# BaZzz01010101/ReflaxMan

Measured on AMD Instinct MI355X. Metric: Mrays/sec at 3840×2160 depth-8; max per-channel |Δ| vs CPU reference, higher is better.
Workload: dtype f32; 1 GPU; C3 synth16: 16 spheres + 4 textured triangles + sun, 3840x2160, depth 8, 1 spp; scene=synth16, width=3840, height=2160, depth=8, spp=1, parallelism=single-gpu

## Files before the change

include/rfx.h:

```cpp
#ifndef RFX_H
#define RFX_H
#include <stddef.h>
#include <stdint.h>

#ifdef __cplusplus
extern "C" {
#endif

#define RFX_ABI_VERSION 5

typedef enum {
  RFX_OK = 0,
  RFX_ERR_ARG = -1,
  RFX_ERR_HIP = -2,
  RFX_ERR_STATE = -3,
  RFX_ERR_IO = -4,
  RFX_ERR_RNG = -5,
  RFX_ERR_NODEV = -6
} rfx_status;

enum { RFX_METAL = 0, RFX_DIELECTRIC = 1 };

typedef struct rfx_scene rfx_scene;
typedef struct rfx_renderer rfx_renderer;

int rfx_abi_version(void);
const char *rfx_last_error(void);
enum { RFX_BUILD_PRIM_LARGE = 1, RFX_BUILD_PRIM_SSAA = 2, RFX_BUILD_PRIM_LANES = 4, RFX_BUILD_ONE_LIGHT = 8 };
int rfx_build_options(void);

rfx_scene *rfx_scene_create(float diff_r, float diff_g, float diff_b, float diff_power);
void rfx_scene_destroy(rfx_scene *scene);
int rfx_scene_add_sphere(rfx_scene *scene, const float center[3], float radius, int material_type,
                         const float rgb[3], float reflectivity, float transparency);
int rfx_scene_add_triangle(rfx_scene *scene, const float v1[3], const float v2[3], const float v3[3],
                           int material_type, const float rgb[3], float reflectivity, float transparency);
int rfx_scene_add_mesh(rfx_scene *scene, const float *vertices, uint32_t n_vertices, const uint32_t *indices,
                       uint32_t n_triangles, int material_type, const float rgb[3], float reflectivity,
                       float transparency);
int rfx_scene_add_plane(rfx_scene *scene, const float pos[3], const float norm[3], int material_type,
                        const float rgb[3], float reflectivity, float transparency);
int rfx_scene_plane_count(const rfx_scene *scene);
int rfx_triangle_set_texture(rfx_scene *scene, int object_index, int texture_index, const float uv[6]);
int rfx_scene_add_light(rfx_scene *scene, const float origin[3], float radius, const float rgb[3], float power);
int rfx_scene_add_texture_argb(rfx_scene *scene, uint32_t width, uint32_t height, const uint32_t *argb);
int rfx_scene_add_texture_file(rfx_scene *scene, const char *path, int *loaded);
int rfx_scene_set_skybox_file(rfx_scene *scene, const char *path);
int rfx_scene_set_skybox_argb(rfx_scene *scene, uint32_t width, uint32_t height, const uint32_t *argb);
int rfx_scene_counts(const rfx_scene *scene, int *spheres, int *triangles, int *lights, int *textures);
int rfx_scene_tri_bvh_dump(const rfx_scene *scene, int32_t counts[5], float *boxes, int32_t *children,
                           int32_t *leaf_ids, int32_t *residual);
int rfx_scene_set_tri_mates(rfx_scene *scene, int on);
int rfx_scene_tri_mates(const rfx_scene *scene, int32_t *leader, float *plane);

void rfx_camera_view(const float eye[3], const float at[3], float view[9]);
float rfx_camera_rz(uint32_t width, float fov);

int rfx_tga_load(const char *path, uint32_t *width, uint32_t *height, uint32_t *argb, size_t capacity);
int rfx_tga_save(const char *path, uint32_t width, uint32_t height, const uint32_t *argb);
int rfx_bmp_save(const char *path, uint32_t width, uint32_t height, const uint32_t *argb);
void rfx_argb_from_rgb(const float *rgb, size_t pixels, uint32_t *argb);

int rfx_renderer_create(rfx_renderer **out, int device);
void rfx_renderer_destroy(rfx_renderer *r);
int rfx_renderer_device(const rfx_renderer *r);
int rfx_renderer_set_stream(rfx_renderer *r, void *hip_stream);
int rfx_renderer_set_scene(rfx_renderer *r, const rfx_scene *scene);
int rfx_renderer_set_tile_order(rfx_renderer *r, int mode);
int rfx_renderer_set_regroup(rfx_renderer *r, int park_after);
int rfx_renderer_set_regroup_sort(rfx_renderer *r, int on);
int rfx_renderer_bounce_form(const rfx_renderer *r);
int rfx_renderer_set_tri_accel(rfx_renderer *r, int mode);
typedef struct {
  int32_t tri_nodes, tri_depth;
  int32_t tri_leaf_size;
  int32_t tri_in_leaves;
  int32_t tri_residual;
  int32_t sph_nodes, sph_depth;
  int32_t narrow_tri_bvh;
} rfx_accel_info;
int rfx_renderer_accel_info(const rfx_renderer *r, rfx_accel_info *out);
int rfx_renderer_set_prim_masks(rfx_renderer *r, int mode);
int rfx_renderer_set_prim_exact(rfx_renderer *r, int on);
int rfx_renderer_get_prim_masks(rfx_renderer *r, uint64_t *host, uint64_t capacity, uint64_t *words);
int rfx_renderer_set_rng(rfx_renderer *r, uint32_t sphere_seed, uint32_t jitter_seed);
int rfx_renderer_get_rng(rfx_renderer *r, uint32_t *sphere_seed, uint32_t *jitter_seed);

typedef struct {
  float eye[3];
  float view[9];
  float fov;
  uint32_t width, height;
  int32_t reflect_num;
  int32_t sample_num;
  int32_t additive;
  int32_t additive_counter;
  uint32_t row_block;
  uint32_t rank, nranks;
  uint64_t pixel_begin;
  uint64_t pixel_end;
  uint64_t span_begin;
  uint64_t span_end;
} rfx_frame;

uint32_t rfx_strip_rows(uint32_t height, uint32_t row_block, uint32_t rank, uint32_t nranks);
uint32_t rfx_strip_row_to_y(uint32_t r, uint32_t row_block, uint32_t rank, uint32_t nranks);

#define RFX_NCOUNTERS 40
int rfx_render_frame(rfx_renderer *r, const rfx_frame *frame, float *d_rgb, uint32_t *d_argb,
                     uint64_t *d_counters, void *stream);
int rfx_renderer_set_launch_traces(rfx_renderer *r, uint64_t max_traces);
int rfx_renderer_set_rng_prepass(rfx_renderer *r, int mode);
int rfx_renderer_prepass_form(const rfx_renderer *r);
uint32_t rfx_rng_triple_index(uint32_t state);
uint32_t rfx_rng_seq_blocks(void);

int rfx_frame_rng_blocks(rfx_renderer *r, const rfx_frame *frame, uint32_t nslices, uint64_t *blocks_per_slice);
int rfx_frame_rng_count(rfx_renderer *r, const rfx_frame *frame, uint32_t slice, uint32_t nslices,
                        uint32_t *d_blk_counts, void *stream);
int rfx_render_frame_counted(rfx_renderer *r, const rfx_frame *frame, uint32_t nslices, const uint32_t *d_blk_counts,
                             float *d_rgb, uint32_t *d_argb, uint64_t *d_counters, void *stream);
int rfx_render_frame_counted_ev(rfx_renderer *r, const rfx_frame *frame, uint32_t nslices,
                                const uint32_t *d_blk_counts, float *d_rgb, uint32_t *d_argb, uint64_t *d_counters,
                                void *stream, void *emitted_event);

int rfx_frame_rng_emit(rfx_renderer *r, const rfx_frame *frame, uint32_t nslices, const uint32_t *d_blk_counts,
                       void *stream, void *emitted_event);
int rfx_render_frame_emitted(rfx_renderer *r, const rfx_frame *frame, float *d_rgb, uint32_t *d_argb,
                             uint64_t *d_counters, void *stream);
int rfx_frame_rng_discard(rfx_renderer *r);
int rfx_frame_rng_pending(rfx_renderer *r, uint32_t *frame_start);

int rfx_trace_rays(rfx_renderer *r, const float *d_rays, uint64_t n, int32_t reflect_num, uint32_t raster_width,
                   float *d_rgb, uint32_t *d_argb, uint64_t *d_counters, void *stream);
int rfx_trace_rays_host(rfx_renderer *r, const float *rays, uint64_t n, int32_t reflect_num, uint32_t raster_width,
                        float *rgb, uint32_t *argb, uint64_t *counters);
int rfx_frame_rng_rewind(rfx_renderer *r);

typedef struct {
  int32_t *object;
  float   *distance;
  float   *point;
  float   *normal;
  float   *reflected;
  float   *colour;
} rfx_hit_planes;
int rfx_query_hits(rfx_renderer *r, const float *d_rays, uint64_t n, uint32_t raster_width,
                   const rfx_hit_planes *out, void *stream);
int rfx_query_occluded(rfx_renderer *r, const float *d_rays, const int32_t *d_skip, uint64_t n,
                       uint32_t raster_width, uint8_t *d_occluded, void *stream);
int rfx_query_hits_host(rfx_renderer *r, const float *rays, uint64_t n, uint32_t raster_width,
                        const rfx_hit_planes *out );
int rfx_query_occluded_host(rfx_renderer *r, const float *rays, const int32_t *skip, uint64_t n,
                            uint32_t raster_width, uint8_t *occluded);

typedef struct {
  const float   *d_lo;
  const int32_t *d_after;
  const float   *d_hi;
} rfx_ray_span;
int rfx_query_hits_span(rfx_renderer *r, const float *d_rays, const rfx_ray_span *span , uint64_t n,
                        uint32_t raster_width, const rfx_hit_planes *out, void *stream);
int rfx_query_occluded_span(rfx_renderer *r, const float *d_rays, const int32_t *d_skip,
                            const rfx_ray_span *span , uint64_t n, uint32_t raster_width,
                            uint8_t *d_occluded, void *stream);
int rfx_query_hits_span_ordered(rfx_renderer *r, const float *d_rays, const rfx_ray_span *span ,
                                const uint32_t *d_order, uint64_t n, const rfx_hit_planes *out, void *stream);
int rfx_query_occluded_span_ordered(rfx_renderer *r, const float *d_rays, const int32_t *d_skip,
                                    const rfx_ray_span *span , const uint32_t *d_order, uint64_t n,
                                    uint8_t *d_occluded, void *stream);
int rfx_query_hits_span_host(rfx_renderer *r, const float *rays, const rfx_ray_span *span ,
                             uint64_t n, uint32_t raster_width, const rfx_hit_planes *out );
int rfx_query_occluded_span_host(rfx_renderer *r, const float *rays, const int32_t *skip,
                                 const rfx_ray_span *span , uint64_t n,
                                 uint32_t raster_width, uint8_t *occluded);

#define RFX_ORDER_CELL_BITS 4
#define RFX_ORDER_DIR_BITS 10
#define RFX_ORDER_TILE 4096
int rfx_renderer_order_box(const rfx_renderer *r, float lo[3], float scale[3]);
int rfx_rays_order(rfx_renderer *r, const float *d_rays, uint64_t n, uint32_t *d_order, uint32_t *d_keys ,
                   void *stream);
int rfx_rays_order_host(rfx_renderer *r, const float *rays, uint64_t n, uint32_t *order, uint32_t *keys );
int rfx_trace_rays_ordered(rfx_renderer *r, const float *d_rays, const uint32_t *d_order, uint64_t n,
                           int32_t reflect_num, float *d_rgb, uint32_t *d_argb, void *stream);
int rfx_query_hits_ordered(rfx_renderer *r, const float *d_rays, const uint32_t *d_order, uint64_t n,
                           const rfx_hit_planes *out, void *stream);
int rfx_query_occluded_ordered(rfx_renderer *r, const float *d_rays, const int32_t *d_skip, const uint32_t *d_order,
                               uint64_t n, uint8_t *d_occluded, void *stream);

typedef struct rfx_group rfx_group;
int rfx_group_create(rfx_group **out, const int *devices, int n);
void rfx_group_destroy(rfx_group *g);
int rfx_group_size(const rfx_group *g);
rfx_renderer *rfx_group_renderer(rfx_group *g, int member);
int rfx_group_set_scene(rfx_group *g, const rfx_scene *scene);
int rfx_group_set_bands(rfx_group *g, uint32_t height, const uint32_t *bounds);
int rfx_group_get_bands(const rfx_group *g, uint32_t *bounds);
int rfx_group_render_frame(rfx_group *g, const rfx_frame *frame, float *d_rgb, uint32_t *d_argb, void *stream);

int rfx_renderer_set_timing(rfx_renderer *r, int enable);
int rfx_renderer_get_timing(rfx_renderer *r, double *prepass_ms, double *trace_ms, uint64_t *frames);

int rfx_render_frame_host(rfx_renderer *r, const rfx_frame *frame, float *rgb, uint32_t *argb,
                          uint64_t *counters);

int rfx_device_alloc(rfx_renderer *r, size_t bytes, void **dptr);
int rfx_device_free(rfx_renderer *r, void *dptr);
int rfx_memcpy_d2h(rfx_renderer *r, void *dst, const void *src, size_t bytes);
int rfx_memcpy_h2d(rfx_renderer *r, void *dst, const void *src, size_t bytes);
int rfx_memcpy_d2d(rfx_renderer *r, void *dst, const void *src, size_t bytes);
int rfx_synchronize(rfx_renderer *r);

int rfx_rand_dirs(rfx_renderer *r, uint32_t seed, uint64_t n, float *out3, uint32_t *seed_out);

int rfx_kat_objects(rfx_renderer *r, const float *rays, const int32_t *objects, uint64_t n, float *out);
int rfx_kat_texels(rfx_renderer *r, int texture, const float *in, uint64_t n, float *out);
int rfx_kat_powf(rfx_renderer *r, const float *xy, uint64_t n, float *out);
int rfx_kat_argb(rfx_renderer *r, const float *rgb, uint64_t n, uint32_t *out);
int rfx_kat_powf_cube(rfx_renderer *r, uint64_t counts[2]);
int rfx_kat_div(rfx_renderer *r, uint64_t first, uint64_t n, uint64_t counts[3]);
int rfx_kat_kernarg(rfx_renderer *r, int swapped, uint32_t out[3]);
int rfx_kat_rng_seq_prefix(rfx_renderer *r, uint32_t *prefix);
int rfx_kat_rng_seq_legacy(rfx_renderer *r, uint32_t *counts);

#ifdef __cplusplus
}
#endif
#endif
```

reflaxman_amd/_lib.py:

```python
from __future__ import annotations

import ctypes as C
import os

from . import _build

RFX_OK = 0
RFX_NCOUNTERS = 40
RFX_ABI_VERSION = 5
RFX_ORDER_CELL_BITS, RFX_ORDER_DIR_BITS, RFX_ORDER_TILE = 4, 10, 4096
METAL, DIELECTRIC = 0, 1

_fp = C.POINTER(C.c_float)
_u32p = C.POINTER(C.c_uint32)
_u64p = C.POINTER(C.c_uint64)


class RfxError(RuntimeError):
    pass


class Frame(C.Structure):
    _fields_ = [
        ("eye", C.c_float * 3), ("view", C.c_float * 9), ("fov", C.c_float),
        ("width", C.c_uint32), ("height", C.c_uint32),
        ("reflect_num", C.c_int32), ("sample_num", C.c_int32),
        ("additive", C.c_int32), ("additive_counter", C.c_int32),
        ("row_block", C.c_uint32), ("rank", C.c_uint32), ("nranks", C.c_uint32),
        ("pixel_begin", C.c_uint64), ("pixel_end", C.c_uint64),
        ("span_begin", C.c_uint64), ("span_end", C.c_uint64),
    ]


class AccelInfo(C.Structure):
    _fields_ = [(n, C.c_int32) for n in ("tri_nodes", "tri_depth", "tri_leaf_size", "tri_in_leaves", "tri_residual",
                                         "sph_nodes", "sph_depth", "narrow_tri_bvh")]


class HitPlanes(C.Structure):
    _fields_ = [(n, C.c_void_p) for n in ("object", "distance", "point", "normal", "reflected", "colour")]


class RaySpan(C.Structure):
    _fields_ = [(n, C.c_void_p) for n in ("d_lo", "d_after", "d_hi")]


_i32p = C.POINTER(C.c_int32)

SIGNATURES = [
    ("rfx_abi_version", C.c_int, []),
    ("rfx_last_error", C.c_char_p, []),
    ("rfx_build_options", C.c_int, []),
    ("rfx_scene_create", C.c_void_p, [C.c_float] * 4),
    ("rfx_scene_destroy", None, [C.c_void_p]),
    ("rfx_scene_add_sphere", C.c_int, [C.c_void_p, _fp, C.c_float, C.c_int, _fp, C.c_float, C.c_float]),
    ("rfx_scene_add_triangle", C.c_int, [C.c_void_p, _fp, _fp, _fp, C.c_int, _fp, C.c_float, C.c_float]),
    ("rfx_scene_add_mesh", C.c_int, [C.c_void_p, _fp, C.c_uint32, _u32p, C.c_uint32, C.c_int, _fp, C.c_float, C.c_float]),
    ("rfx_scene_tri_bvh_dump", C.c_int, [C.c_void_p, _i32p, _fp, _i32p, _i32p, _i32p]),
    ("rfx_scene_set_tri_mates", C.c_int, [C.c_void_p, C.c_int]),
    ("rfx_scene_tri_mates", C.c_int, [C.c_void_p, _i32p, _fp]),
    ("rfx_scene_add_plane", C.c_int, [C.c_void_p, _fp, _fp, C.c_int, _fp, C.c_float, C.c_float]),
    ("rfx_scene_plane_count", C.c_int, [C.c_void_p]),
    ("rfx_triangle_set_texture", C.c_int, [C.c_void_p, C.c_int, C.c_int, _fp]),
    ("rfx_scene_add_light", C.c_int, [C.c_void_p, _fp, C.c_float, _fp, C.c_float]),
    ("rfx_scene_add_texture_argb", C.c_int, [C.c_void_p, C.c_uint32, C.c_uint32, _u32p]),
    ("rfx_scene_add_texture_file", C.c_int, [C.c_void_p, C.c_char_p, C.POINTER(C.c_int)]),
    ("rfx_scene_set_skybox_file", C.c_int, [C.c_void_p, C.c_char_p]),
    ("rfx_scene_set_skybox_argb", C.c_int, [C.c_void_p, C.c_uint32, C.c_uint32, _u32p]),
    ("rfx_scene_counts", C.c_int, [C.c_void_p] + [C.POINTER(C.c_int)] * 4),
    ("rfx_camera_view", None, [_fp, _fp, _fp]),
    ("rfx_camera_rz", C.c_float, [C.c_uint32, C.c_float]),
    ("rfx_tga_load", C.c_int, [C.c_char_p, _u32p, _u32p, _u32p, C.c_size_t]),
    ("rfx_tga_save", C.c_int, [C.c_char_p, C.c_uint32, C.c_uint32, _u32p]),
    ("rfx_bmp_save", C.c_int, [C.c_char_p, C.c_uint32, C.c_uint32, _u32p]),
    ("rfx_argb_from_rgb", None, [_fp, C.c_size_t, _u32p]),
    ("rfx_renderer_create", C.c_int, [C.POINTER(C.c_void_p), C.c_int]),
    ("rfx_renderer_destroy", None, [C.c_void_p]),
    ("rfx_renderer_device", C.c_int, [C.c_void_p]),
    ("rfx_renderer_set_stream", C.c_int, [C.c_void_p, C.c_void_p]),
    ("rfx_renderer_set_scene", C.c_int, [C.c_void_p, C.c_void_p]),
    ("rfx_renderer_set_rng", C.c_int, [C.c_void_p, C.c_uint32, C.c_uint32]),
    ("rfx_renderer_get_rng", C.c_int, [C.c_void_p, _u32p, _u32p]),
    ("rfx_strip_rows", C.c_uint32, [C.c_uint32] * 4),
    ("rfx_strip_row_to_y", C.c_uint32, [C.c_uint32] * 4),
    ("rfx_render_frame", C.c_int, [C.c_void_p, C.POINTER(Frame), C.c_void_p, C.c_void_p, C.c_void_p, C.c_void_p]),
    ("rfx_render_frame_host", C.c_int, [C.c_void_p, C.POINTER(Frame), _fp, _u32p, _u64p]),
    ("rfx_frame_rng_blocks", C.c_int, [C.c_void_p, C.POINTER(Frame), C.c_uint32, _u64p]),
    ("rfx_frame_rng_count", C.c_int, [C.c_void_p, C.POINTER(Frame), C.c_uint32, C.c_uint32, C.c_void_p, C.c_void_p]),
    ("rfx_render_frame_counted", C.c_int, [C.c_void_p, C.POINTER(Frame), C.c_uint32, C.c_void_p, C.c_void_p,
                                           C.c_void_p, C.c_void_p, C.c_void_p]),
    ("rfx_render_frame_counted_ev", C.c_int, [C.c_void_p, C.POINTER(Frame), C.c_uint32, C.c_void_p, C.c_void_p,
                                              C.c_void_p, C.c_void_p, C.c_void_p, C.c_void_p]),
    ("rfx_frame_rng_emit", C.c_int, [C.c_void_p, C.POINTER(Frame), C.c_uint32, C.c_void_p, C.c_void_p, C.c_void_p]),
    ("rfx_render_frame_emitted", C.c_int, [C.c_void_p, C.POINTER(Frame), C.c_void_p, C.c_void_p, C.c_void_p,
                                           C.c_void_p]),
    ("rfx_frame_rng_discard", C.c_int, [C.c_void_p]),
    ("rfx_frame_rng_pending", C.c_int, [C.c_void_p, _u32p]),
    ("rfx_frame_rng_rewind", C.c_int, [C.c_void_p]),
    ("rfx_trace_rays", C.c_int, [C.c_void_p, C.c_void_p, C.c_uint64, C.c_int32, C.c_uint32, C.c_void_p, C.c_void_p,
                                 C.c_void_p, C.c_void_p]),
    ("rfx_trace_rays_host", C.c_int, [C.c_void_p, _fp, C.c_uint64, C.c_int32, C.c_uint32, _fp, _u32p, _u64p]),
    ("rfx_query_hits", C.c_int, [C.c_void_p, C.c_void_p, C.c_uint64, C.c_uint32, C.POINTER(HitPlanes), C.c_void_p]),
    ("rfx_query_hits_host", C.c_int, [C.c_void_p, _fp, C.c_uint64, C.c_uint32, C.POINTER(HitPlanes)]),
    ("rfx_query_occluded", C.c_int, [C.c_void_p, C.c_void_p, C.c_void_p, C.c_uint64, C.c_uint32, C.c_void_p, C.c_void_p]),
    ("rfx_query_occluded_host", C.c_int, [C.c_void_p, _fp, _i32p, C.c_uint64, C.c_uint32, C.POINTER(C.c_uint8)]),
    ("rfx_query_hits_span", C.c_int, [C.c_void_p, C.c_void_p, C.POINTER(RaySpan), C.c_uint64, C.c_uint32,
                                      C.POINTER(HitPlanes), C.c_void_p]),
    ("rfx_query_occluded_span", C.c_int, [C.c_void_p, C.c_void_p, C.c_void_p, C.POINTER(RaySpan), C.c_uint64, C.c_uint32,
                                          C.c_void_p, C.c_void_p]),
    ("rfx_query_hits_span_ordered", C.c_int, [C.c_void_p, C.c_void_p, C.POINTER(RaySpan), C.c_void_p, C.c_uint64,
                                              C.POINTER(HitPlanes), C.c_void_p]),
    ("rfx_query_occluded_span_ordered", C.c_int, [C.c_void_p, C.c_void_p, C.c_void_p, C.POINTER(RaySpan), C.c_void_p,
                                                  C.c_uint64, C.c_void_p, C.c_void_p]),
    ("rfx_query_hits_span_host", C.c_int, [C.c_void_p, _fp, C.POINTER(RaySpan), C.c_uint64, C.c_uint32,
                                           C.POINTER(HitPlanes)]),
    ("rfx_query_occluded_span_host", C.c_int, [C.c_void_p, _fp, _i32p, C.POINTER(RaySpan), C.c_uint64, C.c_uint32,
                                               C.POINTER(C.c_uint8)]),
    ("rfx_renderer_order_box", C.c_int, [C.c_void_p, _fp, _fp]),
    ("rfx_rays_order", C.c_int, [C.c_void_p, C.c_void_p, C.c_uint64, C.c_void_p, C.c_void_p, C.c_void_p]),
    ("rfx_rays_order_host", C.c_int, [C.c_void_p, _fp, C.c_uint64, _u32p, _u32p]),
    ("rfx_trace_rays_ordered", C.c_int, [C.c_void_p, C.c_void_p, C.c_void_p, C.c_uint64, C.c_int32, C.c_void_p,
                                         C.c_void_p, C.c_void_p]),
    ("rfx_query_hits_ordered", C.c_int, [C.c_void_p, C.c_void_p, C.c_void_p, C.c_uint64, C.POINTER(HitPlanes),
                                         C.c_void_p]),
    ("rfx_query_occluded_ordered", C.c_int, [C.c_void_p, C.c_void_p, C.c_void_p, C.c_void_p, C.c_uint64, C.c_void_p,
                                             C.c_void_p]),
    ("rfx_group_create", C.c_int, [C.POINTER(C.c_void_p), C.POINTER(C.c_int), C.c_int]),
    ("rfx_group_destroy", None, [C.c_void_p]),
    ("rfx_group_size", C.c_int, [C.c_void_p]),
    ("rfx_group_renderer", C.c_void_p, [C.c_void_p, C.c_int]),
    ("rfx_group_set_scene", C.c_int, [C.c_void_p, C.c_void_p]),
    ("rfx_group_set_bands", C.c_int, [C.c_void_p, C.c_uint32, _u32p]),
    ("rfx_group_get_bands", C.c_int, [C.c_void_p, _u32p]),
    ("rfx_group_render_frame", C.c_int, [C.c_void_p, C.POINTER(Frame), C.c_void_p, C.c_void_p, C.c_void_p]),
    ("rfx_renderer_set_timing", C.c_int, [C.c_void_p, C.c_int]),
    ("rfx_renderer_set_tile_order", C.c_int, [C.c_void_p, C.c_int]),
    ("rfx_renderer_set_prim_masks", C.c_int, [C.c_void_p, C.c_int]),
    ("rfx_renderer_set_prim_exact", C.c_int, [C.c_void_p, C.c_int]),
    ("rfx_renderer_get_prim_masks", C.c_int, [C.c_void_p, _u64p, C.c_uint64, _u64p]),
    ("rfx_renderer_set_regroup", C.c_int, [C.c_void_p, C.c_int]),
    ("rfx_renderer_set_regroup_sort", C.c_int, [C.c_void_p, C.c_int]),
    ("rfx_renderer_set_launch_traces", C.c_int, [C.c_void_p, C.c_uint64]),
    ("rfx_renderer_bounce_form", C.c_int, [C.c_void_p]),
    ("rfx_renderer_set_rng_prepass", C.c_int, [C.c_void_p, C.c_int]),
    ("rfx_renderer_prepass_form", C.c_int, [C.c_void_p]),
    ("rfx_rng_triple_index", C.c_uint32, [C.c_uint32]),
    ("rfx_rng_seq_blocks", C.c_uint32, []),
    ("rfx_renderer_set_tri_accel", C.c_int, [C.c_void_p, C.c_int]),
    ("rfx_renderer_accel_info", C.c_int, [C.c_void_p, C.POINTER(AccelInfo)]),
    ("rfx_renderer_get_timing", C.c_int, [C.c_void_p, C.POINTER(C.c_double), C.POINTER(C.c_double), _u64p]),
    ("rfx_device_alloc", C.c_int, [C.c_void_p, C.c_size_t, C.POINTER(C.c_void_p)]),
    ("rfx_device_free", C.c_int, [C.c_void_p, C.c_void_p]),
    ("rfx_memcpy_d2h", C.c_int, [C.c_void_p, C.c_void_p, C.c_void_p, C.c_size_t]),
    ("rfx_memcpy_h2d", C.c_int, [C.c_void_p, C.c_void_p, C.c_void_p, C.c_size_t]),
    ("rfx_memcpy_d2d", C.c_int, [C.c_void_p, C.c_void_p, C.c_void_p, C.c_size_t]),
    ("rfx_synchronize", C.c_int, [C.c_void_p]),
    ("rfx_rand_dirs", C.c_int, [C.c_void_p, C.c_uint32, C.c_uint64, _fp, _u32p]),
    ("rfx_kat_objects", C.c_int, [C.c_void_p, _fp, C.POINTER(C.c_int32), C.c_uint64, _fp]),
    ("rfx_kat_texels", C.c_int, [C.c_void_p, C.c_int, _fp, C.c_uint64, _fp]),
    ("rfx_kat_powf", C.c_int, [C.c_void_p, _fp, C.c_uint64, _fp]),
    ("rfx_kat_argb", C.c_int, [C.c_void_p, _fp, C.c_uint64, _u32p]),
    ("rfx_kat_powf_cube", C.c_int, [C.c_void_p, C.POINTER(C.c_uint64)]),
    ("rfx_kat_div", C.c_int, [C.c_void_p, C.c_uint64, C.c_uint64, C.POINTER(C.c_uint64)]),
    ("rfx_kat_kernarg", C.c_int, [C.c_void_p, C.c_int, C.POINTER(C.c_uint32)]),
    ("rfx_kat_rng_seq_prefix", C.c_int, [C.c_void_p, _u32p]),
    ("rfx_kat_rng_seq_legacy", C.c_int, [C.c_void_p, _u32p]),
]

_lib = None


def lib_path() -> str:
    return _build.LIB


def bind(path: str, partial: bool = False):
    L = C.CDLL(os.path.abspath(path))
    for name, res, args in SIGNATURES:
        if partial and not hasattr(L, name):
            continue
        fn = getattr(L, name)
        fn.restype = res
        fn.argtypes = args
    return L


def load(build_if_missing: bool = True):
    global _lib
    if _lib is not None:
        return _lib
    path = _build.LIB
    if build_if_missing:
        try:
            _build.build()
        except Exception as e:
            if not os.path.exists(path):
                raise RfxError(f"librfx.so missing and cannot be built: {e}") from e
    if not os.path.exists(path):
        raise RfxError(f"librfx.so not found at {path}: the HIP renderer is required (no CPU fallback)")
    L = C.CDLL(path)
    for name, res, args in SIGNATURES:
        fn = getattr(L, name)
        fn.restype = res
        fn.argtypes = args
    if L.rfx_abi_version() != RFX_ABI_VERSION:
        raise RfxError("librfx.so ABI version mismatch")
    _lib = L
    return L


def lib_sha256(path: str = None) -> str:
    import hashlib
    with open(path or _build.LIB, "rb") as f:
        return hashlib.sha256(f.read()).hexdigest()


def device_sha256(path: str = None) -> str:
    import hashlib
    import struct
    with open(path or _build.LIB, "rb") as f:
        b = f.read()
    shoff = struct.unpack_from("<Q", b, 0x28)[0]
    shentsize, shnum, shstrndx = struct.unpack_from("<HHH", b, 0x3A)
    secs = [struct.unpack_from("<IIQQQQIIQQ", b, shoff + i * shentsize) for i in range(shnum)]
    names = secs[shstrndx][4]
    for name_off, _, _, _, off, size, *_ in secs:
        if b[names + name_off:b.index(b"\0", names + name_off)] == b".hip_fatbin":
            return hashlib.sha256(b[off:off + size]).hexdigest()
    return None


def check(rc: int, what: str = "") -> int:
    if rc < 0:
        msg = load().rfx_last_error().decode(errors="replace")
        raise RfxError(f"{what or 'rfx call'} failed ({rc}): {msg}")
    return rc


def fptr(a):
    return a.ctypes.data_as(_fp)


def u32ptr(a):
# ... 13 lines not shown
```

reflaxman_amd/csrc/rfx_bounce.h:

```cpp
#pragma once
#include <hip/hip_runtime.h>

#include <cstddef>
#include <type_traits>

#include "rfx_math.h"
#include "rfx_types.h"
#include "rfx_shade_inputs.h"
#include "rfx_queries.h"

#pragma clang fp contract(off)

namespace rfx {

struct Park {
  int after;
  QRay *queue;
  uint32_t *count;
  uint32_t trace, out;
  static constexpr bool kRefill = false;
  __device__ __forceinline__ void ids(uint32_t &t, uint32_t &o) const { t = trace; o = out; }
  __device__ __forceinline__ uint32_t *keys() const { return nullptr; }
  __device__ __forceinline__ BvhGlobal bvh() const { return BvhGlobal{}; }
};

__device__ __forceinline__ uint32_t queue_key(const DevScene &S, v3 o, v3 d)
{
  const auto cell = [](float v, float lo, float s) -> uint32_t {
    return (uint32_t)fminf(fmaxf((v - lo) * s, 0.0f), 7.0f);
  };
  const uint32_t cx = cell(o.x, S.key_lx, S.key_sx), cy = cell(o.y, S.key_ly, S.key_sy), cz = cell(o.z, S.key_lz, S.key_sz);
  uint32_t m = 0;
#pragma unroll
  for (int b = 0; b < 3; ++b)
    m |= (((cx >> b) & 1u) << (3 * b)) | (((cy >> b) & 1u) << (3 * b + 1)) | (((cz >> b) & 1u) << (3 * b + 2));
  const uint32_t oct = (d.x < 0.0f ? 1u : 0u) | (d.y < 0.0f ? 2u : 0u) | (d.z < 0.0f ? 4u : 0u);
  return oct << 9 | m;
}

__shared__ __attribute__((aligned(16))) uint32_t s_out[kWgWaves][256];

#ifndef RFX_NO_LAUNDER
#define RFX_LAUNDER_SCENE
#define RFX_LAUNDER_PARAMS
#endif
#ifdef RFX_LAUNDER_SCENE
typedef const __attribute__((address_space(4))) DevScene *ConstScenePtr;
template <bool ON>
__device__ __forceinline__ const DevScene &launder_scene(const DevScene &S)
{
  if constexpr (!ON) return S;
  ConstScenePtr p = (ConstScenePtr)__builtin_amdgcn_kernarg_segment_ptr();
  asm volatile("" : "+s"(p));
  return *(const DevScene *)p;
}
#define RFX_SCENE_PARAM S_in
#else
#define RFX_SCENE_PARAM S
#endif
constexpr size_t kParamsOff = (sizeof(DevScene) + alignof(FrameParams) - 1) / alignof(FrameParams) * alignof(FrameParams);
struct KernargPair { DevScene S; FrameParams P; };
static_assert(offsetof(KernargPair, S) == 0 && offsetof(KernargPair, P) == kParamsOff,
              "kernel-argument layout: DevScene at offset 0, FrameParams at kParamsOff");
template <class F>
constexpr bool kKernargSig = std::is_same<F, void (*)(DevScene, FrameParams)>::value;
template <bool LAUNDER = true>
__device__ __forceinline__ const FrameParams &kernarg_params()
{
  typedef const __attribute__((address_space(4))) char *KP;
  KP p = (KP)__builtin_amdgcn_kernarg_segment_ptr();
  if constexpr (LAUNDER) asm volatile("" : "+s"(p));
  return *(const FrameParams *)(const __attribute__((address_space(4))) FrameParams *)(p + kParamsOff);
}

template <bool STATS, bool CULL, bool MANYL, bool SMALL, bool PLANES, bool PARK, class PK, bool ONEL = false,
          bool TBVH = false>
__device__ __forceinline__ col trace_from(const DevScene &RFX_SCENE_PARAM, v3 origin, v3 ray, col mulc, col pix, int refl,
                                          int depth, v3 rd, const float *lut, Cnt &cnt, bool valid, const PK &park,
                                          bool &parked, const uint64_t *pm_tile = nullptr, bool pm_shadow = true)
{
#ifdef RFX_LAUNDER_SCENE
  const DevScene &S = S_in;
#endif
  bool seg0 = pm_tile != nullptr;
  parked = false;
  if (valid && refl == 0) RFX_CNT(C_RAYS);
  const Tabs<SMALL> T{S};
  bool alive = valid && refl < depth;
  int occ_hint = -1;
#ifdef RFX_DEBUG_SEGS
  int nseg = 0;
#endif
  RFX_PROF_BEGIN(P_SEG);
  while (__ballot(alive))
  {
#ifdef RFX_DEBUG_SEGS
    if (alive) ++nseg;
#endif
#ifdef RFX_LAUNDER_SCENE
    const DevScene &S = launder_scene<!SMALL>(S_in);
    const Tabs<SMALL> T{S};
#endif
    Hit h;
    if constexpr (SMALL)
    {
      uint64_t om = S.cull_valid;
      if constexpr (CULL)
      {
        if (seg0)
          om = pm_tile[0];
        else
        {
          const Bundle B = make_bundle(origin, ray, alive);
          if (B.ok) om = cull_small(T.cull(), S.cull_valid, B);
          RFX_CULL_STAT(0, B.ok, __ballot(alive), om, S.cull_valid);
        }
      }
      if (alive) closest_hit_small<STATS, PLANES>(S, origin, ray, om, h, cnt);
      else h.obj = -1;
    }
    else
    {
      Bundle B;
      if constexpr (CULL) B = make_bundle(origin, ray, alive);
      closest_hit<STATS, PLANES, TBVH>(S, origin, ray, alive, CULL ? &B : nullptr, h, cnt, park.bvh());
    }
    const bool hit = alive && h.obj >= 0;
    v3 drop = origin, norm = mk(0.0f, 0.0f, 0.0f);
    RFX_PROF_BEGIN(P_WIN);
    if (hit)
    {
      drop = add(origin, mul(ray, h.t));
      if (h.kind == 0)
      {
        RFX_CNT(C_HIT_SPH);
        const SphereGeo g = T.sph_geo(h.i);
        norm = sub(drop, mk(g.cx, g.cy, g.cz));
      }
      else if (!PLANES || h.kind == 1)
      {
        RFX_CNT(C_HIT_TRI);
        const TriShade sh = T.tri_shade(h.i);
        norm = mk(sh.nx, sh.ny, sh.nz);
      }
      else
      {
        RFX_CNT(C_HIT_PLN);
        const PlaneGeo g = S.pln_geo[h.i];
        norm = mk(g.nx, g.ny, g.nz);
      }
    }
    RFX_PROF_END(P_WIN);
    const int skip_sph = h.kind == 0 ? h.i : -1, skip_tri = h.kind == 1 ? h.i : -1;
    const int skip_pln = PLANES && h.kind == 2 ? h.i : -1;
    MatRec m{0.0f, 0.0f, 0.0f, 0.0f};
    int diel = 0;
    v3 reflv = mk(0.0f, 0.0f, 0.0f);
    float rayLen = 0.0f, normLen = 0.0f, reflectLen = 0.0f;
    col sumL = mkc(0.0f, 0.0f, 0.0f), sumS = mkc(0.0f, 0.0f, 0.0f);
    for (int base = 0;; base += 32)
    {
      RFX_PROF_BEGIN(P_SHADOW);
      uint32_t lit = 0;
      const int nl = ONEL ? 1 : min(32, S.n_light - base);
      for (int q = 0; q < nl; ++q)
      {
        const LightRec L = S.lights[base + q];
        bool facing = false;
        v3 sray = mk(0.0f, 0.0f, 0.0f);
        if (hit)
        {
          RFX_CNT(C_L_EVAL);
          const v3 dtl = sub(mk(L.ox, L.oy, L.oz), drop);
          if (dot(dtl, norm) > kVerySmall)
          {
            RFX_CNT(C_L_FACING);
            facing = true;
            sray = add(dtl, mul(rd, L.radius));
          }
        }
        if (__ballot(facing))
        {
          if constexpr (SMALL)
          {
            uint64_t om = S.cull_valid;
            if constexpr (CULL)
            {
              if (!MANYL && seg0 && pm_shadow && q < kPrimLights)
                om = pm_tile[1 + q];
              else
              {
                const Bundle SB = make_bundle(drop, sray, facing);
                if (SB.ok) om = cull_small(T.cull(), S.cull_valid, SB);
                RFX_CULL_STAT(1, SB.ok, __ballot(facing), om, S.cull_valid);
              }
            }
            if (facing && !occluded_small<STATS, PLANES>(S, drop, sray, skip_sph, skip_tri, skip_pln, om, cnt))
              lit |= 1u << q;
          }
          else
          {
            Bundle SB;
            if constexpr (CULL) SB = make_bundle(drop, sray, facing);
            const bool occ = occluded<STATS, PLANES, TBVH>(S, drop, sray, facing, skip_sph, skip_tri, skip_pln,
                                                     CULL ? &SB : nullptr, cnt, park.bvh(), &occ_hint);
            if (facing && !occ) lit |= 1u << q;
          }
        }
      }
      RFX_PROF_END(P_SHADOW);
      RFX_PROF_BEGIN(P_LIGHT);
      if (hit)
      {
        if (!MANYL || base == 0)
        {
          if (h.kind == 0)
          {
            m = T.sph_mat(h.i);
            diel = T.sph_info(2 * h.i + 1);
          }
          else if (PLANES && h.kind == 2)
          {
            m = S.pln_mat[h.i];
            diel = S.pln_geo[h.i].dielectric;
          }
          else
          {
            const TriShade sh = T.tri_shade(h.i);
            m = T.tri_mat(h.i);
            diel = sh.dielectric;
            if (sh.tex >= 0)
            {
              const col c = tri_texel<STATS>(S, sh, h.u, h.v, lut, cnt);
              m.r = c.r; m.g = c.g; m.b = c.b;
            }
          }
          reflv = reflect(mul(ray, h.t), norm);
          rayLen = len(ray); normLen = len(norm); reflectLen = len(reflv);
        }
        for (int q = 0; q < nl; ++q)
        {
          if (!((lit >> q) & 1u)) continue;
          RFX_CNT(C_L_LIT);
          const LightRec L = S.lights[base + q];
          const v3 dtl = sub(mk(L.ox, L.oy, L.oz), drop);
          const float dlen = len(dtl);
          float aa = dlen * normLen;
          const float cosl = (aa > kVerySmall) ? qdiv(dot(dtl, norm), aa) : 0.0f;
          const col lc = mkc(L.r, L.g, L.b);
          if (L.power > kVerySmall) sumL = cadd(sumL, cscale(cscale(lc, cosl), L.power));
          aa = sqlen(dtl);
          const float ang = (aa > kVerySmall) ? 1.0f - qdiv(L.radius * L.radius, aa) : 0.0f;
          if (ang > 0)
          {
            RFX_CNT(C_L_SPEC);
            const v3 dlr = add(normalized(dtl), mul(rd, 1.0f - m.refl));
            aa = len(dlr) * reflectLen;
            float sc = (aa > kVerySmall) ? qdiv(dot(dlr, reflv), aa) : 0.0f;
            sc = clampf(sc + (1.0f - sqrt_rn(ang)), 0.0f, 1.0f);
            if (sc > kVerySmall && L.radius > kVerySmall)
            {
              RFX_CNT(C_L_POW);
              const float sp = powf_dev(sc, 1 + qdiv(3 * m.refl * dlen, L.radius)) * m.refl;
              sumS = cadd(sumS, cscale(lc, sp));
            }
          }
        }
      }
      RFX_PROF_END(P_LIGHT);
      if (!MANYL || base + 32 >= S.n_light) break;
    }
    if (hit)
    {
      RFX_PROF_BEGIN(P_MAT);
      sumL = cadd(mkc(S.amb_r, S.amb_g, S.amb_b), sumL);
      const col color = mkc(m.r, m.g, m.b);
      col fin;
      if (diel)
      {
        RFX_CNT(C_DIELECTRIC);
        const float aa = rayLen * normLen;
        const float cosA = (aa > kVerySmall) ? clampf(qdiv(dot(ray, neg(norm)), aa), 0.0f, 1.0f) : 0.0f;
        const float r = 0.2f + 0.8f * powf3_dev(1.0f - cosA);
        fin = cadd(cmul(cscale(color, 1.0f - r), sumL), sumS);
        fin = cmul(fin, mulc);
        mulc = cscale(mulc, r);
      }
      else
      {
        RFX_CNT(C_METAL);
        const float r = 0.8f;
        fin = cadd(cmul(cscale(color, 1.0f - r), sumL), sumS);
        fin = cmul(fin, mulc);
        mulc = cmul(mulc, cscale(color, r));
      }
      pix = cclamp(cadd(pix, fin));
      RFX_PROF_END(P_MAT);
      if (mulc.r < 0.01f && mulc.g < 0.01f && mulc.b < 0.01f)
        alive = false;
      else
      {
        RFX_CNT(C_CONTINUE);
        origin = drop;
        ray = add(normalized(reflv), mul(rd, 1.0f - m.refl));
        if (++refl >= depth) alive = false;
      }
    }
    else if (alive)
    {
      RFX_CNT(C_SKY);
      RFX_PROF_BEGIN(P_SKY);
      pix = cclamp(cadd(pix, cmul(cmul(mulc, skybox_texel<STATS>(S, ray, lut, cnt)), mkc(S.env_r, S.env_g, S.env_b))));
      RFX_PROF_END(P_SKY);
      alive = false;
    }
    seg0 = false;
    if constexpr (!STATS && PARK)
    {
      if (refl == park.after && __ballot(alive))
      {
        const uint64_t pm = __ballot(alive);
        uint32_t base = 0;
        if (__lane_id() == (uint32_t)(__ffsll((long long)pm) - 1)) base = atomicAdd(park.count, (uint32_t)__popcll(pm));
        base = __builtin_amdgcn_readlane(base, __ffsll((long long)pm) - 1);
        if (alive)
        {
          QRay q;
          q.ox = origin.x; q.oy = origin.y; q.oz = origin.z; q.dx = ray.x;
          q.dy = ray.y; q.dz = ray.z; q.mr = mulc.r; q.mg = mulc.g;
          q.mb = mulc.b; q.pr = pix.r; q.pg = pix.g; q.pb = pix.b;
          uint32_t qt, qo;
          park.ids(qt, qo);
          q.trace = qt; q.out = qo; q.refl = (uint32_t)refl; q.pad = 0;
          const uint32_t slot = base + (uint32_t)__popcll(pm & ((1ull << __lane_id()) - 1ull));
          park.queue[slot] = q;
          if (uint32_t *keys = park.keys()) keys[slot] = queue_key(S, origin, ray);
          parked = true;
          alive = false;
        }
      }
    }
    if constexpr (PK::kRefill) park.refill(alive, origin, ray, mulc, pix, refl, rd);
  }
  RFX_PROF_END(P_SEG);
#ifdef RFX_DEBUG_SEGS
  return mkc((float)nseg, 0.0f, 0.0f);
#else
  return pix;
#endif
}

template <bool STATS, bool CULL, bool MANYL, bool SMALL, bool PLANES, bool ONEL = false, bool TBVH = false>
__device__ __forceinline__ col trace(const DevScene &S, v3 origin, v3 ray, int depth, v3 rd, const float *lut,
                                     Cnt &cnt, bool valid, const uint64_t *pm_tile = nullptr, bool pm_shadow = true)
{
  bool parked;
  return trace_from<STATS, CULL, MANYL, SMALL, PLANES, false, Park, ONEL, TBVH>(S, origin, ray, mkc(1.0f, 1.0f, 1.0f), mkc(0.0f, 0.0f, 0.0f), 0,
                                                       depth, rd, lut, cnt, valid, Park{0, nullptr, nullptr, 0, 0},
                                                       parked, pm_tile, pm_shadow);
}

}
```

reflaxman_amd/csrc/rfx_bundle.h:

```cpp
#pragma once
#include <hip/hip_runtime.h>

#include "rfx_math.h"
#include "rfx_types.h"

#pragma clang fp contract(off)

namespace rfx {

constexpr float kCullRel = 2e-3f;

struct Bundle {
  float cx, cy, cz, rw;
  float ax, ay, az, cosa, sina;
  bool ok;
};

__device__ __forceinline__ float lane_bcast(float v, int lane)
{
  return __int_as_float(__builtin_amdgcn_readlane(__float_as_int(v), lane));
}

__device__ __forceinline__ float wave_max_nonneg(float v)
{
  uint32_t u = __float_as_uint(v);
  u = max(u, (uint32_t)__builtin_amdgcn_update_dpp(0, (int)u, 0x111, 0xf, 0xf, false));
  u = max(u, (uint32_t)__builtin_amdgcn_update_dpp(0, (int)u, 0x112, 0xf, 0xf, false));
  u = max(u, (uint32_t)__builtin_amdgcn_update_dpp(0, (int)u, 0x114, 0xf, 0xf, false));
  u = max(u, (uint32_t)__builtin_amdgcn_update_dpp(0, (int)u, 0x118, 0xf, 0xf, false));
  u = max(u, (uint32_t)__builtin_amdgcn_update_dpp(0, (int)u, 0x142, 0xa, 0xf, false));
  u = max(u, (uint32_t)__builtin_amdgcn_update_dpp(0, (int)u, 0x143, 0xc, 0xf, false));
  return __int_as_float(__builtin_amdgcn_readlane((int)u, 63));
}

__device__ __forceinline__ float cdot(float ax, float ay, float az, float bx, float by, float bz)
{
#if RFX_CULL_FMA
  return __builtin_fmaf(az, bz, __builtin_fmaf(ay, by, ax * bx));
#else
  return ax * bx + ay * by + az * bz;
#endif
}

__device__ __forceinline__ Bundle make_bundle(v3 o, v3 d, bool live)
{
  Bundle B;
  const int ref = __ffsll((long long)__ballot(live)) - 1;
  B.cx = lane_bcast(o.x, ref); B.cy = lane_bcast(o.y, ref); B.cz = lane_bcast(o.z, ref);
  const float dx = lane_bcast(d.x, ref), dy = lane_bcast(d.y, ref), dz = lane_bcast(d.z, ref);
  const float inv = __builtin_amdgcn_rsqf(cdot(dx, dy, dz, dx, dy, dz));
  B.ax = dx * inv; B.ay = dy * inv; B.az = dz * inv;
  const float ex = o.x - B.cx, ey = o.y - B.cy, ez = o.z - B.cz;
  const float e2 = cdot(ex, ey, ez, ex, ey, ez);
  const float cosl = cdot(d.x, d.y, d.z, B.ax, B.ay, B.az) * __builtin_amdgcn_rsqf(cdot(d.x, d.y, d.z, d.x, d.y, d.z));
  const float dev = 1.0f - cosl;
  const bool bad = live && !(e2 <= 1.0e30f && dev >= -0.5f && dev <= 2.5f);
  const float e2m = wave_max_nonneg(live ? e2 : 0.0f);
  const float devm = wave_max_nonneg(live ? fmaxf(dev, 0.0f) : 0.0f);
  B.rw = __builtin_amdgcn_sqrtf(e2m) * 1.0001f;
  B.cosa = 1.0f - devm - 4e-6f;
  B.sina = __builtin_amdgcn_sqrtf(fmaxf(1.0f - B.cosa * B.cosa, 0.0f) + 1e-7f) * 1.001f;
  B.ok = __ballot(bad) == 0 && B.cosa > 0.1f && B.rw <= 1.0e15f;
  return B;
}

__device__ __forceinline__ Bundle make_bundle_ball(v3 o, v3 d, float R, bool live)
{
  Bundle B;
  const int ref = __ffsll((long long)__ballot(live)) - 1;
  B.cx = lane_bcast(o.x, ref); B.cy = lane_bcast(o.y, ref); B.cz = lane_bcast(o.z, ref);
  const float dx = lane_bcast(d.x, ref), dy = lane_bcast(d.y, ref), dz = lane_bcast(d.z, ref);
  const float inv = __builtin_amdgcn_rsqf(dx * dx + dy * dy + dz * dz);
  B.ax = dx * inv; B.ay = dy * inv; B.az = dz * inv;
  const float ex = o.x - B.cx, ey = o.y - B.cy, ez = o.z - B.cz;
  const float e2 = ex * ex + ey * ey + ez * ez;
  const float d2 = d.x * d.x + d.y * d.y + d.z * d.z;
  const float id = __builtin_amdgcn_rsqf(d2);
  const float ca = fminf((d.x * B.ax + d.y * B.ay + d.z * B.az) * id, 1.0f);
  const float sa = __builtin_amdgcn_sqrtf(fmaxf(1.0f - ca * ca, 0.0f));
  const float sb = fminf(R * id * 1.001f, 1.0f), cb = __builtin_amdgcn_sqrtf(fmaxf(1.0f - sb * sb, 0.0f));
  const float cosl = ca * cb - sa * sb;
  const float dev = 1.0f - cosl;
  const bool bad = live && !(e2 <= 1.0e30f && dev >= -0.5f && dev <= 2.5f && sb < 0.5f);
  const float e2m = wave_max_nonneg(live ? e2 : 0.0f);
  const float devm = wave_max_nonneg(live ? fmaxf(dev, 0.0f) : 0.0f);
  B.rw = __builtin_amdgcn_sqrtf(e2m) * 1.0001f;
  B.cosa = 1.0f - devm - 4e-6f;
  B.sina = __builtin_amdgcn_sqrtf(fmaxf(1.0f - B.cosa * B.cosa, 0.0f) + 1e-7f) * 1.001f;
  B.ok = __ballot(bad) == 0 && B.cosa > 0.1f && B.rw <= 1.0e15f;
  return B;
}

__device__ __forceinline__ Bundle make_bundle_quad(v3 o, const v3 (&d)[4], bool live)
{
  Bundle B;
  const int ref = __ffsll((long long)__ballot(live)) - 1;
  B.cx = lane_bcast(o.x, ref); B.cy = lane_bcast(o.y, ref); B.cz = lane_bcast(o.z, ref);
  const float dx = lane_bcast(d[0].x, ref), dy = lane_bcast(d[0].y, ref), dz = lane_bcast(d[0].z, ref);
  const float inv = __builtin_amdgcn_rsqf(dx * dx + dy * dy + dz * dz);
  B.ax = dx * inv; B.ay = dy * inv; B.az = dz * inv;
  const float ex = o.x - B.cx, ey = o.y - B.cy, ez = o.z - B.cz;
  const float e2 = ex * ex + ey * ey + ez * ez;
  float dev = 0.0f;
  bool bad = false;
#pragma unroll
  for (int k = 0; k < 4; ++k)
  {
    const v3 v = d[k];
    const float cosl = (v.x * B.ax + v.y * B.ay + v.z * B.az) * __builtin_amdgcn_rsqf(v.x * v.x + v.y * v.y + v.z * v.z);
    const float dk = 1.0f - cosl;
    bad = bad || !(dk >= -0.5f && dk <= 2.5f);
    dev = fmaxf(dev, dk);
  }
  bad = live && (bad || !(e2 <= 1.0e30f));
  const float e2m = wave_max_nonneg(live ? e2 : 0.0f);
  const float devm = wave_max_nonneg(live ? fmaxf(dev, 0.0f) : 0.0f);
  B.rw = __builtin_amdgcn_sqrtf(e2m) * 1.0001f;
  B.cosa = 1.0f - devm - 4e-6f;
  B.sina = __builtin_amdgcn_sqrtf(fmaxf(1.0f - B.cosa * B.cosa, 0.0f) + 1e-7f) * 1.001f;
  B.ok = __ballot(bad) == 0 && B.cosa > 0.1f && B.rw <= 1.0e15f;
  return B;
}

__device__ __forceinline__ uint64_t cull_chunk(const Bound *bound, int first, int n, const Bundle &B)
{
  const int l = (int)(threadIdx.x & 63u);
  bool keep = false;
  if (l < n)
  {
    const Bound g = bound[first + l];
    const float vx = g.x - B.cx, vy = g.y - B.cy, vz = g.z - B.cz;
    const float L2 = cdot(vx, vy, vz, vx, vy, vz);
    const float L = __builtin_amdgcn_sqrtf(L2);
#if RFX_CULL_FMA
    const float rp = __builtin_fmaf(kCullRel, L + B.rw, g.r + B.rw);
    const float va = cdot(vx, vy, vz, B.ax, B.ay, B.az);
    const float lim = __builtin_fmaf(B.cosa, __builtin_amdgcn_sqrtf(fmaxf(__builtin_fmaf(-rp, rp, L2), 0.0f)), -(B.sina * rp));
#else
    const float rp = g.r + B.rw + kCullRel * (L + B.rw);
    const float va = cdot(vx, vy, vz, B.ax, B.ay, B.az);
    const float lim = B.cosa * __builtin_amdgcn_sqrtf(fmaxf(L2 - rp * rp, 0.0f)) - B.sina * rp;
#endif
    keep = !(L > rp && va < lim);
  }
  return __ballot(keep);
}

__device__ __forceinline__ bool tri_footprint_misses(const CullTri &q, float side, float an, const Bundle &B)
{
  const float h = fabsf(side), anp = side > 0.0f ? -an : an;
  const float snp = __builtin_amdgcn_sqrtf(fmaxf(1.0f - anp * anp, 0.0f));
  const float ndmin = anp * B.cosa - snp * B.sina;
  if (!(h > B.rw * 1.01f + 1e-4f && ndmin > 0.1f)) return false;
  const float ind = __builtin_amdgcn_rcpf(ndmin) * 1.001f, ian = __builtin_amdgcn_rcpf(anp) * 1.001f;
  const float tp = h * ian * (1.0f / 1.001f);
  const float px = B.cx + tp * B.ax - q.v0x, py = B.cy + tp * B.ay - q.v0y, pz = B.cz + tp * B.az - q.v0z;
  const float chord = __builtin_amdgcn_sqrtf(fmaxf(2.0f - 2.0f * B.cosa, 0.0f)) * 1.001f;
  const float R = (h * chord * (1.0f + ian) * ind + B.rw * (1.0f + ind) + 1e-4f * tp) * 1.001f + 1e-6f;
  const float cvx = B.cx - q.v0x, cvy = B.cy - q.v0y, cvz = B.cz - q.v0z;
  const float mag = __builtin_amdgcn_sqrtf(cvx * cvx + cvy * cvy + cvz * cvz) * 1.001f + B.rw + (h + B.rw) * ind;
  const float m = 1e-2f * mag + 1e-6f;
  const float u0 = q.gux * px + q.guy * py + q.guz * pz, v0 = q.gvx * px + q.gvy * py + q.gvz * pz;
  return u0 + (R + m) * q.nu < 0.0f || v0 + (R + m) * q.nv < 0.0f ||
         u0 + v0 - R * q.nuv - m * (q.nu + q.nv) > 1.0f;
}

template <bool FOOT = false>
__device__ __forceinline__ uint64_t cull_small(const CullRec *tab, uint64_t valid, const Bundle &B,
                                               const CullTri *ttab = nullptr)
{
  const CullRec g = tab[threadIdx.x & 63u];
  const float vx = g.x - B.cx, vy = g.y - B.cy, vz = g.z - B.cz;
// ... 36 lines not shown
```

reflaxman_amd/csrc/rfx_config.h:

```cpp
#pragma once

#ifndef RFX_DIV_FAST
#define RFX_DIV_FAST 1
#endif
#ifndef RFX_DIV_SINGLE
#define RFX_DIV_SINGLE 0
#endif

#ifndef RFX_BVH_LEAF_PAIRS
#define RFX_BVH_LEAF_PAIRS 4
#endif
#ifndef RFX_TRI_BVH
#define RFX_TRI_BVH 1
#endif
#ifndef RFX_TRI_BVH_LEAF
#define RFX_TRI_BVH_LEAF 4
#endif
#ifndef RFX_TRI_BVH_AUTO_MIN
#define RFX_TRI_BVH_AUTO_MIN 128
#endif
#ifndef RFX_TRI_BVH_NARROW_MIN
#define RFX_TRI_BVH_NARROW_MIN (1 << 30)
#endif

#if !defined(RFX_WAVES_PER_EU) && defined(RFX_LANES_WAVES_PER_EU) && defined(RFX_UNIT_LANES_FAST)
#define RFX_WAVES_PER_EU RFX_LANES_WAVES_PER_EU
#endif
#ifndef RFX_WAVES_PER_EU
#define RFX_WAVES_PER_EU 7
#endif
#ifndef RFX_WG_WAVES
#define RFX_WG_WAVES 2
#endif
#ifndef RFX_TRI_MATES
#define RFX_TRI_MATES 2
#endif
#ifndef RFX_CULL_FMA
#define RFX_CULL_FMA 1
#endif
#ifndef RFX_NARROW_BUNDLE_COS
#define RFX_NARROW_BUNDLE_COS 0.9995f
#endif
#ifndef RFX_OCC_HINT
#define RFX_OCC_HINT 1
#endif
#ifndef RFX_ONE_LIGHT
#define RFX_ONE_LIGHT 1
#endif
#ifndef RFX_SSAA_LANES
#define RFX_SSAA_LANES 1
#endif
#ifndef RFX_SSAA_CHANNEL_SUM
#define RFX_SSAA_CHANNEL_SUM 1
#endif
#ifndef RFX_PRIM_SSAA
#define RFX_PRIM_SSAA 0
#endif
#ifndef RFX_PRIM_LANES
#define RFX_PRIM_LANES 1
#endif
#ifndef RFX_PRIM_CHUNKS
#define RFX_PRIM_CHUNKS 1
#endif
#ifndef RFX_NOCULL_MAX_TILES
#define RFX_NOCULL_MAX_TILES 0
#endif

#ifndef RFX_RNG_INT_ACCEPT
#define RFX_RNG_INT_ACCEPT 1
#endif
#ifndef RFX_RNG_TICKET
#define RFX_RNG_TICKET 1
#endif
#ifndef RFX_LOOKBACK_SLEEP
#define RFX_LOOKBACK_SLEEP 1
#endif
#ifndef RFX_LOOKBACK_SPINS
#define RFX_LOOKBACK_SPINS (1u << 22)
#endif
#ifndef RFX_SCAN_TILES
#define RFX_SCAN_TILES 2
#endif
#ifndef RFX_SCAN_EMIT_BLOCKS
#define RFX_SCAN_EMIT_BLOCKS 16384
#endif
#ifndef RFX_RNG_FUSED
#define RFX_RNG_FUSED 1
#endif
#ifndef RFX_RNG_FUSED_MAX_BLOCKS
#define RFX_RNG_FUSED_MAX_BLOCKS 256
#endif
#ifndef RFX_RNG_SEQ
#define RFX_RNG_SEQ 1
#endif
#ifndef RFX_RNG_SEQ_SPLIT
#define RFX_RNG_SEQ_SPLIT 1
#endif
#ifndef RFX_RNG_SEQ_MIN_BLOCKS
#define RFX_RNG_SEQ_MIN_BLOCKS 0
#endif

#ifndef RFX_TILE_ORDER_DEFAULT
#define RFX_TILE_ORDER_DEFAULT 1
#endif
#ifndef RFX_TILE_ORDER_MIN_TILES
#define RFX_TILE_ORDER_MIN_TILES 49152
#endif
#ifndef RFX_TILE_SORT_MAIN
#define RFX_TILE_SORT_MAIN 1
#endif
#ifndef RFX_TILE_SORT_EVERY
#define RFX_TILE_SORT_EVERY 16
#endif
#ifndef RFX_PARK_AFTER
#define RFX_PARK_AFTER 2
#endif
#ifndef RFX_QUEUE_SORT
#define RFX_QUEUE_SORT 0
// ... 13 lines not shown
```

reflaxman_amd/csrc/rfx_kat.cpp:

```cpp
#include <algorithm>
#include <string>
#include <vector>

#include "rfx_internal.h"

using namespace rfx;

static int named(const char *who, int rc)
{
  const std::string cause = rfx_last_error();
  return fail(rc, "%s: %s", who, cause.c_str());
}

template <class T>
static int kat_buffer(DevBuf<T> &dev, size_t n, const T *src)
{
  int rc;
  if ((rc = dev.reserve(n ? n : 1)) < 0) return rc;
  if (src && n) HIP_CHECK(hipMemcpy(dev, src, n * sizeof(T), hipMemcpyHostToDevice));
  return RFX_OK;
}

static int kat_run(rfx_renderer *r, int what, int tex, const void *in, size_t in_elems, const int32_t *objs,
                   uint64_t n, void *out, size_t out_elems)
{
  RCHECK(set_dev(r));
  if (n >= (1ull << 31)) return fail(RFX_ERR_ARG, "kat: n too large");
  DevBuf<float> d_in, d_out;
  DevBuf<int32_t> d_obj;
  RCHECK(kat_buffer(d_in, in_elems, (const float *)in));
  if (objs) RCHECK(kat_buffer(d_obj, (size_t)n, objs));
  RCHECK(kat_buffer(d_out, out_elems, (const float *)nullptr));
  hipError_t e = launch_kat(what, r->dev, tex, d_in, d_obj, (uint32_t)n, d_out, r->stream);
  if (e == hipSuccess) e = hipStreamSynchronize(r->stream);
  if (e == hipSuccess) e = hipMemcpy(out, d_out, out_elems * 4, hipMemcpyDeviceToHost);
  return e == hipSuccess ? RFX_OK : fail(RFX_ERR_HIP, "kat: %s", hipGetErrorString(e));
}

extern "C" int rfx_kat_objects(rfx_renderer *r, const float *rays, const int32_t *objects, uint64_t n, float *out)
{
  if (!r || (n && (!rays || !objects || !out))) return fail(RFX_ERR_ARG, "kat_objects: bad args");
  if (!r->has_scene) return fail(RFX_ERR_STATE, "kat_objects: no scene uploaded");
  for (uint64_t i = 0; i < n; ++i)
    if (objects[i] < 0 || objects[i] >= r->dev.n_obj) return fail(RFX_ERR_ARG, "kat_objects: object %d", objects[i]);
  return kat_run(r, 0, 0, rays, (size_t)n * 6, objects, n, out, (size_t)n * 15);
}

extern "C" int rfx_kat_texels(rfx_renderer *r, int texture, const float *in, uint64_t n, float *out)
{
  if (!r || (n && (!in || !out))) return fail(RFX_ERR_ARG, "kat_texels: bad args");
  if (!r->has_scene) return fail(RFX_ERR_STATE, "kat_texels: no scene uploaded");
  if (texture >= r->dev.n_tex) return fail(RFX_ERR_ARG, "kat_texels: texture %d", texture);
  return kat_run(r, 1, texture, in, (size_t)n * (texture >= 0 ? 2 : 3), nullptr, n, out, (size_t)n * 3);
}

extern "C" int rfx_kat_powf(rfx_renderer *r, const float *xy, uint64_t n, float *out)
{
  if (!r || (n && (!xy || !out))) return fail(RFX_ERR_ARG, "kat_powf: bad args");
  return kat_run(r, 2, 0, xy, (size_t)n * 2, nullptr, n, out, (size_t)n);
}

extern "C" int rfx_kat_argb(rfx_renderer *r, const float *rgb, uint64_t n, uint32_t *out)
{
  if (!r || (n && (!rgb || !out))) return fail(RFX_ERR_ARG, "kat_argb: bad args");
  return kat_run(r, 3, 0, rgb, (size_t)n * 3, nullptr, n, out, (size_t)n);
}

extern "C" int rfx_kat_powf_cube(rfx_renderer *r, uint64_t counts[2])
{
  if (!r || !counts) return fail(RFX_ERR_ARG, "kat_powf_cube: bad args");
  DevBuf<unsigned long long> d;
  int rc;
  if ((rc = d.reserve(2)) < 0) return named("kat_powf_cube", rc);
  hipError_t e = hipMemsetAsync(d, 0, 2 * sizeof(unsigned long long), r->stream);
  for (uint64_t first = 0; e == hipSuccess && first <= 0x3f800000ull; first += 1ull << 28)
    e = launch_kat_powf_cube((uint32_t)first, (uint32_t)std::min<uint64_t>(1ull << 28, 0x3f800001ull - first), d, r->stream);
  unsigned long long h[2] = {0, 0};
  if (e == hipSuccess) e = hipStreamSynchronize(r->stream);
  if (e == hipSuccess) e = hipMemcpy(h, d, sizeof(h), hipMemcpyDeviceToHost);
  if (e != hipSuccess) return fail(RFX_ERR_HIP, "kat_powf_cube: %s", hipGetErrorString(e));
  counts[0] = h[0];
  counts[1] = h[1];
  return RFX_OK;
}

extern "C" int rfx_kat_div(rfx_renderer *r, uint64_t first, uint64_t n, uint64_t counts[3])
{
  if (!r || !counts) return fail(RFX_ERR_ARG, "kat_div: bad args");
  RCHECK(set_dev(r));
  DevBuf<unsigned long long> d;
  int rc;
  if ((rc = d.reserve(3)) < 0) return named("kat_div", rc);
  hipError_t e = hipMemsetAsync(d, 0, 3 * sizeof(unsigned long long), r->stream);
  for (uint64_t k = 0; e == hipSuccess && k < n; k += 1ull << 28)
    e = launch_kat_div(first + k, (uint32_t)std::min<uint64_t>(1ull << 28, n - k), d, r->stream);
  unsigned long long h[3] = {0, 0, 0};
  if (e == hipSuccess) e = hipStreamSynchronize(r->stream);
  if (e == hipSuccess) e = hipMemcpy(h, d, sizeof(h), hipMemcpyDeviceToHost);
  if (e != hipSuccess) return fail(RFX_ERR_HIP, "kat_div: %s", hipGetErrorString(e));
  for (int i = 0; i < 3; ++i) counts[i] = h[i];
  return RFX_OK;
}

extern "C" uint32_t rfx_rng_seq_blocks(void) { return rng_seq_blocks(); }

extern "C" int rfx_kat_rng_seq_prefix(rfx_renderer *r, uint32_t *prefix)
{
  if (!r || !prefix) return fail(RFX_ERR_ARG, "kat_rng_seq_prefix: bad args");
  RCHECK(set_dev(r));
  RCHECK(ensure_seq_table(r, r->stream));
  HIP_CHECK(hipStreamSynchronize(r->stream));
  HIP_CHECK(hipMemcpy(prefix, r->seq_p, ((size_t)rng_seq_blocks() + 1) * sizeof(uint32_t), hipMemcpyDeviceToHost));
  return RFX_OK;
}

extern "C" int rfx_kat_rng_seq_legacy(rfx_renderer *r, uint32_t *counts)
{
  if (!r || !counts) return fail(RFX_ERR_ARG, "kat_rng_seq_legacy: bad args");
  RCHECK(set_dev(r));
  const uint64_t nb = rng_seq_blocks();
  std::vector<uint32_t> jump(2 * (256 + nb));
  rng_jump_table(nb, jump.data());
  DevBuf<uint32_t> d_jump, d_cnt, d_origin;
  int rc;
  if ((rc = d_jump.reserve(jump.size())) < 0 || (rc = d_cnt.reserve(nb)) < 0 || (rc = d_origin.reserve(1)) < 0)
    return named("kat_rng_seq_legacy", rc);
  hipError_t e = hipMemcpy(d_jump, jump.data(), jump.size() * sizeof(uint32_t), hipMemcpyHostToDevice);
  if (e == hipSuccess) e = hipMemset(d_origin, 0, sizeof(uint32_t));
  if (e == hipSuccess) e = launch_rng_count(d_origin, d_jump, d_cnt, 0, nb, nullptr, r->stream);
  if (e == hipSuccess) e = hipStreamSynchronize(r->stream);
  if (e == hipSuccess) e = hipMemcpy(counts, d_cnt, nb * sizeof(uint32_t), hipMemcpyDeviceToHost);
  if (e != hipSuccess) return fail(RFX_ERR_HIP, "kat_rng_seq_legacy: %s", hipGetErrorString(e));
  return RFX_OK;
}

extern "C" int rfx_kat_kernarg(rfx_renderer *r, int swapped, uint32_t out[3])
{
  if (!r || !out) return fail(RFX_ERR_ARG, "kat_kernarg: bad args");
  if (!r->has_scene) return fail(RFX_ERR_STATE, "kat_kernarg: no scene uploaded");
  RCHECK(set_dev(r));
  FrameParams P;
  uint32_t *w = (uint32_t *)&P;
// ... 12 lines not shown
```

reflaxman_amd/csrc/rfx_kernels.hip:

```cpp
#include "rfx_trace.h"
#include "rfx_prim_cull.h"

#include <vector>

#pragma clang fp contract(off)

namespace rfx {

constexpr int kLptThreads = 1024, kLptBuckets = 256, kLptGroups = 64;

__device__ __forceinline__ uint32_t lpt_key(const uint32_t *cost, uint32_t i)
{
  const uint32_t c = max(cost[i], 1u);
  const uint32_t e = 31u - (uint32_t)__clz(c);
  const uint32_t m = e >= 3u ? (c >> (e - 3u)) & 7u : (c << (3u - e)) & 7u;
  return (uint32_t)(kLptBuckets - 1) - min(e * 8u + m, (uint32_t)(kLptBuckets - 1));
}

__global__ __launch_bounds__(kLptThreads) void lpt_hist(const uint32_t *cost, uint32_t n, uint32_t chunk, uint32_t *hist)
{
  __shared__ uint32_t h[kLptBuckets];
  for (uint32_t b = threadIdx.x; b < kLptBuckets; b += kLptThreads) h[b] = 0;
  __syncthreads();
  const uint32_t i0 = blockIdx.x * chunk, i1 = min(n, i0 + chunk);
// ... 821 lines not shown
  if (kind == 0)
  {
    const SphereGeo g = S.sph_geo[idx];
    SpherePair p;
    p.cx[0] = g.cx; p.cy[0] = g.cy; p.cz[0] = g.cz; p.r2[0] = g.sq_radius;
    p.cx[1] = 0.0f; p.cy[1] = 0.0f; p.cz[1] = 0.0f; p.r2[1] = -INFINITY;
    f2 b, d;
    pair_bd(p, o, k, b, d);
    hit = pair_may_hit(b, d) && sphere_tail<false, false>(b.x, d.x, ray, k, t, sq, cnt);
    any = pair_may_hit(b, d) && sphere_tail<false, true>(b.x, d.x, ray, k, t2, sq2, cnt);
    if (hit)
    {
      drop = add(o, mul(ray, t));
      norm = sub(drop, mk(g.cx, g.cy, g.cz));
      const MatRec m = S.sph_mat[idx];
      c = mkc(m.r, m.g, m.b);
    }
  }
  else if (kind == 1)
  {
    hit = tri_hit<false, false>(S.tri_geo[idx], o, ray, t, u, v, sq, cnt, k);
    any = tri_hit<false, true>(S.tri_geo[idx], o, ray, t2, u2, v2, sq2, cnt, k);
    if (tri_hit<false, true, true>(S.tri_geo[idx], o, ray, t2, u2, v2, sq2, cnt, k) != any) pre_bad = true;
    if (hit)
    {
      drop = add(o, mul(ray, t));
      const TriShade sh = S.tri_shade[idx];
      norm = mk(sh.nx, sh.ny, sh.nz);
      const MatRec m = S.tri_mat[idx];
      c = sh.tex >= 0 ? tri_texel<false>(S, sh, u, v, lut, cnt) : mkc(m.r, m.g, m.b);
    }
  }
  else
  {
    const PlaneGeo g = S.pln_geo[idx];
    hit = plane_hit<false, false>(g, o, ray, t, sq, cnt, k);
    any = plane_hit<false, true>(g, o, ray, t2, sq2, cnt, k);
    if (hit)
    {
      drop = add(o, mul(ray, t));
      norm = mk(g.nx, g.ny, g.nz);
      const MatRec m = S.pln_mat[idx];
      c = mkc(m.r, m.g, m.b);
    }
  }
  float *w = out + 15 * (size_t)i;
  for (int j = 0; j < 15; ++j) w[j] = 0.0f;
  w[0] = hit ? 1.0f : 0.0f;
  if (hit)
  {
    const v3 rf = reflect(mul(ray, t), norm);
    w[1] = drop.x; w[2] = drop.y; w[3] = drop.z;
    w[4] = norm.x; w[5] = norm.y; w[6] = norm.z;
    w[7] = rf.x; w[8] = rf.y; w[9] = rf.z;
    w[10] = sqrt_rn(sq);
    w[11] = c.r; w[12] = c.g; w[13] = c.b;
  }
  w[14] = pre_bad ? __builtin_nanf("") : any ? 1.0f : 0.0f;
}

__global__ __launch_bounds__(kKatThreads) void kat_texels(DevScene S, int tex, const float *in, uint32_t n, float *out)
{
  __shared__ float lut[256];
  stage_lut(lut);
  __syncthreads();
  const uint32_t i = blockIdx.x * kKatThreads + threadIdx.x;
  if (i >= n) return;
  Cnt cnt;
  const col c = tex >= 0 ? texel_uv<false>(S, tex, in[2 * (size_t)i], in[2 * (size_t)i + 1], lut, cnt)
                         : skybox_texel<false>(S, mk(in[3 * (size_t)i], in[3 * (size_t)i + 1], in[3 * (size_t)i + 2]), lut, cnt);
  out[3 * (size_t)i] = c.r; out[3 * (size_t)i + 1] = c.g; out[3 * (size_t)i + 2] = c.b;
}

__global__ __launch_bounds__(kKatThreads) void kat_powf(const float *xy, uint32_t n, float *out)
{
  stage_powf_tables();
  __syncthreads();
  const uint32_t i = blockIdx.x * kKatThreads + threadIdx.x;
  if (i < n)
  {
    const float x = xy[2 * (size_t)i], y = xy[2 * (size_t)i + 1];
    out[i] = y == 3.0f ? powf3_dev(x) : powf_dev(x, y);
  }
}

__global__ __launch_bounds__(kKatThreads) void kat_powf_cube(uint32_t first, uint32_t n, unsigned long long *counts)
{
  stage_powf_tables();
  __syncthreads();
  const uint32_t i = blockIdx.x * kKatThreads + threadIdx.x;
  bool bad = false, slow = false;
  if (i < n)
  {
    const float x = __uint_as_float(first + i);
    float p;
    slow = !powf_cube_fast(x, p);
    bad = __float_as_uint(powf3_dev(x)) != __float_as_uint(powf_dev(x, 3.0f));
  }
  const uint64_t mb = __ballot(bad), ms = __ballot(slow);
  if ((threadIdx.x & 63u) == 0 && (mb | ms))
  {
    atomicAdd(&counts[0], (unsigned long long)__popcll(mb));
    atomicAdd(&counts[1], (unsigned long long)__popcll(ms));
  }
}

__device__ __forceinline__ uint32_t kat_mix(uint64_t x)
{
  x ^= x >> 33; x *= 0xff51afd7ed558ccdull; x ^= x >> 33; x *= 0xc4ceb9fe1a85ec53ull; x ^= x >> 33;
  return (uint32_t)x;
}
__device__ __forceinline__ float kat_float(uint32_t sign, int32_t e, uint32_t mant)
{
  return __uint_as_float((sign & 1u) << 31 | (uint32_t)(e + 127) << 23 | (mant & 0x7FFFFFu));
}
__device__ __forceinline__ bool kat_same(float x, float y)
{
  return __float_as_uint(x) == __float_as_uint(y) || (x != x && y != y);
}
__global__ __launch_bounds__(kKatThreads) void kat_div(uint64_t first, uint32_t n, unsigned long long *counts)
{
  const uint32_t i = blockIdx.x * kKatThreads + threadIdx.x;
  uint32_t bad = 0, fast = 0, seen = 0;
  if (i < n)
  {
    const uint64_t k = first + i;
    const uint32_t h0 = kat_mix(k), h1 = kat_mix(k ^ 0x9E3779B97F4A7C15ull), h2 = kat_mix(k * 3 + 1);
    float a, b;
    switch (h0 & 7u)
    {
      case 0: a = __uint_as_float(h1); b = __uint_as_float(h2); break;
      case 1:
      {
        b = kat_float(h1 >> 31, (int32_t)(h1 % 151u) - 45, h2);
        a = b * kat_float(h2 >> 31, (int32_t)((h0 >> 3) % 133u) - 66, h1 >> 5);
        break;
      }
      case 2:
      {
        const float edge = (h1 & 1u) ? 0x1p100f : 0x1p-40f;
        b = __uint_as_float(__float_as_uint(edge) + (int32_t)((h1 >> 1) % 7u) - 3) * ((h1 & 2u) ? -1.0f : 1.0f);
        const int32_t qe = (h2 % 3u == 0) ? -60 : (h2 % 3u == 1) ? 60 : 0;
        a = b * kat_float(h2 >> 31, qe + (int32_t)((h2 >> 2) % 5u) - 2, h0 >> 3);
        break;
      }
      case 3:
      {
        const uint32_t m = h1 % 3u;
        a = m == 0 ? ((h1 & 8u) ? -0.0f : 0.0f) : m == 1 ? __uint_as_float((h1 & 0x807FFFFFu)) : kat_float(h1 >> 31, -126 + (int32_t)(h2 % 40u), h2);
        b = kat_float(h2 >> 31, (int32_t)(h0 % 141u) - 40, h1 >> 3);
        break;
      }
      case 4: b = kat_float(h1 >> 31, (int32_t)((h1 >> 1) % 3u) - 1, h2); a = kat_float(h2 >> 31, (int32_t)(h0 % 253u) - 126, h1 >> 4); break;
      case 5: a = kat_float(h1 >> 31, (int32_t)(h0 % 253u) - 126, h2); b = kat_float(h2 >> 31, (int32_t)(h1 % 253u) - 126, h0); break;
      case 6: b = kat_float(h1 >> 31, (int32_t)(h0 % 141u) - 40, h2); a = b * __uint_as_float(0x3f800000u + (h2 & 0xFu) - 8u); break;
      default: b = kat_float(h1 >> 31, (int32_t)(h0 % 253u) - 126, 0u); a = kat_float(h2 >> 31, (int32_t)(h1 % 253u) - 126, h2 >> 1); break;
    }
    const float q = div_rn(a, b);
    bool ok;
    (void)div_fast(a, div_prep(b), ok);
    const float a2 = __uint_as_float(__float_as_uint(a) ^ (h2 & 0x807F0000u)), a3 = b * -0.5f;
    const v3 v = mk(a, a2, a3), nv = normalized(v);
    const float l = len(v);
    const bool sv = l > kVerySmall;
    const float rx = sv ? v.x / l : v.x, ry = sv ? v.y / l : v.y, rz = sv ? v.z / l : v.z;
    const float den = fabsf(b) + kVerySmall, p = fabsf(a) <= den ? a : copysignf(den, a) * 0.75f;
// ... 150 lines not shown
  for (int j = 0; j < 32; ++j)
  {
    hdr[kSeqPow2 + 2 * j] = a;
    hdr[kSeqPow2 + 2 * j + 1] = c;
    c = a * c + c;
    a = a * a;
  }
  if (!state) return;
  uint32_t s = 0;
  for (uint32_t b = 0; b < kSeqBlocks; ++b)
  {
    state[b] = s;
    s = ab * s + cb;
  }
}

uint32_t rng_seq_index_of(uint32_t s)
{
  uint32_t hdr[kSeqHeader];
  rng_seq_tables(hdr, nullptr);
  return seq_index_of(s, hdr + kSeqPow2);
}

hipError_t launch_rng_seq_build(const uint32_t *d_hdr, const uint32_t *d_state, uint32_t *d_p, uint32_t *d_tiles,
                                hipStream_t st)
{
  const uint32_t ntiles = kSeqBlocks / kScanTileCounts;
  hipLaunchKernelGGL(rng_seq_count, dim3(kSeqBlocks), dim3(kRngBlock), 0, st, d_state, d_hdr, d_p);
  hipLaunchKernelGGL(rng_tile_sums, dim3(ntiles), dim3(kTileSumThreads), 0, st, (const uint32_t *)d_p,
                     (uint64_t)kSeqBlocks, d_tiles, d_tiles + ntiles);
  hipLaunchKernelGGL(rng_seq_scan, dim3(ntiles), dim3(kScanThreads), 0, st, d_p, (const uint32_t *)d_tiles);
  return hipGetLastError();
}

hipError_t launch_rng_locate(const uint32_t *d_seed, const uint32_t *d_hdr, const uint32_t *d_state, const uint32_t *d_p,
                             uint32_t *d_pos, hipStream_t st)
{
  hipLaunchKernelGGL(rng_locate, dim3(1), dim3(kRngBlock), 0, st, d_seed, d_hdr + kSeqPow2, d_state, d_hdr, d_p, d_pos);
  return hipGetLastError();
}

hipError_t launch_rng_emit_seq(const uint32_t *d_pos, const uint32_t *d_hdr, const uint32_t *d_state, const uint32_t *d_p,
                               uint64_t nblk, uint64_t traces, uint32_t *d_rd_state, uint32_t *d_next_seed,
                               uint32_t *d_next_pos, int *d_err, hipStream_t st)
{
  hipLaunchKernelGGL(rng_emit_seq, dim3((uint32_t)nblk), dim3(kRngBlock), 0, st, d_pos, d_state, d_hdr, d_p, traces,
                     d_rd_state, d_next_seed, d_next_pos, d_err);
  return hipGetLastError();
}

static void launch_mode_cfg(bool stats, int mode, int cfg, dim3 grid, const DevScene &S, const FrameParams &P,
                            hipStream_t st)
{
  if (mode == kModeBlock) (stats ? launch_trace_block_stats : launch_trace_block_fast)(cfg, grid, S, P, st);
  else if (mode == kModePlain)
  {
    if (stats) launch_trace_plain_stats(cfg, grid, S, P, st);
    else if (P.park_after > 0) launch_trace_plain_park(cfg, grid, S, P, st);
    else launch_trace_plain_fast(cfg, grid, S, P, st);
  }
  else if (mode == kModeSsaaLanes) (stats ? launch_trace_lanes_stats : launch_trace_lanes_fast)(cfg, grid, S, P, st);
  else if (mode == kModeSsaaChunks) (stats ? launch_trace_chunks_stats : launch_trace_chunks_fast)(cfg, grid, S, P, st);
  else (stats ? launch_trace_ssaa_stats : launch_trace_ssaa_fast)(cfg, grid, S, P, st);
}

static dim3 kat_grid(uint32_t n) { return dim3((n + kKatThreads - 1) / kKatThreads); }

hipError_t launch_kat_kernarg(const DevScene &S, const FrameParams &P, int swapped, uint32_t *out, hipStream_t st)
{
  if (swapped) hipLaunchKernelGGL(kat_kernarg_swapped, dim3(1), dim3(64), 0, st, P, S, out);
  else hipLaunchKernelGGL(kat_kernarg, dim3(1), dim3(64), 0, st, S, P, out);
  return hipGetLastError();
}

hipError_t launch_kat(int what, const DevScene &S, int tex, const void *in, const int32_t *objs, uint32_t n, void *out,
                      hipStream_t st)
{
  if (!n) return hipSuccess;
  switch (what)
  {
    case 0: hipLaunchKernelGGL(kat_objects, kat_grid(n), dim3(kKatThreads), 0, st, S, (const float *)in, objs, n, (float *)out); break;
    case 1: hipLaunchKernelGGL(kat_texels, kat_grid(n), dim3(kKatThreads), 0, st, S, tex, (const float *)in, n, (float *)out); break;
    case 2: hipLaunchKernelGGL(kat_powf, kat_grid(n), dim3(kKatThreads), 0, st, (const float *)in, n, (float *)out); break;
    default: hipLaunchKernelGGL(kat_argb, kat_grid(n), dim3(kKatThreads), 0, st, (const float *)in, n, (uint32_t *)out); break;
  }
  return hipGetLastError();
}

hipError_t launch_kat_div(uint64_t first, uint32_t n, unsigned long long *counts, hipStream_t st)
{
  if (!n) return hipSuccess;
  hipLaunchKernelGGL(kat_div, kat_grid(n), dim3(kKatThreads), 0, st, first, n, counts);
  return hipGetLastError();
}

hipError_t launch_kat_powf_cube(uint32_t first, uint32_t n, unsigned long long *counts, hipStream_t st)
{
  if (!n) return hipSuccess;
  hipLaunchKernelGGL(kat_powf_cube, kat_grid(n), dim3(kKatThreads), 0, st, first, n, counts);
  return hipGetLastError();
}

static int trace_mode(const FrameParams &P)
{
  if (P.ss < 0) return kModeBlock;
  if (P.ss == 1 && !P.additive && !P.accumulate) return kModePlain;
  if (!RFX_SSAA_LANES || !ss_lane_block(P.ss)) return kModeSsaa;
  return P.ss > 8 ? kModeSsaaChunks : kModeSsaaLanes;
}

static dim3 trace_grid(const FrameParams &P)
{
  const int mode = trace_mode(P);
  if (mode == kModeSsaaLanes || mode == kModeSsaaChunks)
  {
    const uint32_t bw = ss_lane_block(P.ss);
    return dim3((P.W + kTileWavesX * bw - 1) / (kTileWavesX * bw), (P.grid_rows + kTileWavesY * bw - 1) / (kTileWavesY * bw));
  }
  const uint32_t cols = P.ss < 0 ? (P.W + (uint32_t)(-P.ss) - 1) / (uint32_t)(-P.ss) : P.W;
  return dim3((cols + kTileW - 1) / kTileW, (P.grid_rows + kTileH - 1) / kTileH);
}

uint32_t trace_tiles(const FrameParams &P)
{
  const dim3 g = trace_grid(P);
  return kWgWaves * g.x * g.y;
}

bool trace_lanes(const FrameParams &P)
{
  return trace_mode(P) == kModeSsaaLanes;
}

bool trace_chunks(const FrameParams &P)
{
  return trace_mode(P) == kModeSsaaChunks;
}

hipError_t launch_prim_cull(const DevScene &S, const FrameParams &P, uint64_t *masks, bool narrow, hipStream_t st)
{
  const int nw = narrow ? 1 : 0;
  const dim3 grid = trace_grid(P);
  if (!(S.n_sph <= 32 && S.n_tri <= 32)) return hipErrorInvalidValue;
  if (trace_lanes(P) || trace_chunks(P))
  {
    if (S.n_pln > 0)
      hipLaunchKernelGGL((prim_cull_kernel<true, true>), grid, dim3(kWgThreads), 0, st, S, P, masks, nw);
    else
      hipLaunchKernelGGL((prim_cull_kernel<false, true>), grid, dim3(kWgThreads), 0, st, S, P, masks, nw);
  }
  else if (S.n_pln > 0)
    hipLaunchKernelGGL(prim_cull_kernel<true>, grid, dim3(kWgThreads), 0, st, S, P, masks, nw);
  else
    hipLaunchKernelGGL(prim_cull_kernel<false>, grid, dim3(kWgThreads), 0, st, S, P, masks, nw);
  return hipGetLastError();
}

hipError_t launch_trace(const DevScene &S, const FrameParams &P, bool stats, hipStream_t st)
{
  const dim3 grid = trace_grid(P);
  FrameParams Pt = P;
  Pt.tiles_x = kTileWavesX * grid.x;
  const int mode = trace_mode(P);
  const bool cull = !stats && !(RFX_NOCULL_MAX_TILES > 0 && S.n_sph <= 32 && S.n_tri <= 32 &&
                                trace_tiles(P) <= (uint32_t)RFX_NOCULL_MAX_TILES);
  const int cfg = (S.n_light > 32 ? kCfgManyLights : 0) | (cull ? kCfgCull : 0) |
                  (S.n_sph <= 32 && S.n_tri <= 32 ? kCfgSmall : 0) | (S.n_pln > 0 ? kCfgPlanes : 0) |
                  (S.n_light == 1 && !stats && RFX_ONE_LIGHT ? kCfgOneLight : 0) |
                  (RFX_TRI_BVH && S.tri_bvh != nullptr && !stats ? kCfgTriBvh : 0);
  launch_mode_cfg(stats, mode, cfg, grid, S, Pt, st);
  return hipGetLastError();
}

}
```

reflaxman_amd/csrc/rfx_scene.cpp:

```cpp
#include <math.h>
#include <stdarg.h>
#include <stdio.h>
#include <stdlib.h>
#include <string.h>

#include <algorithm>
#include <array>
#include <cmath>
#include <map>
#include <string>
#include <vector>

#include "rfx_math.h"
#include "rfx_scene.h"

#pragma clang fp contract(off)

using namespace rfx;

static thread_local std::string g_last_error;

int rfx::fail(int code, const char *fmt, ...)
{
  char buf[512];
  va_list ap;
  va_start(ap, fmt);
  vsnprintf(buf, sizeof(buf), fmt, ap);
  va_end(ap);
  g_last_error = buf;
  return code;
}

extern "C" const char *rfx_last_error(void) { return g_last_error.c_str(); }

struct HostTexture { uint32_t w = 0, h = 0; bool loaded = false; std::vector<uint32_t> texels; };
struct HostMat { int dielectric; float r, g, b, refl, transp; };
struct HostSphere { v3 center; float radius, sq_radius; HostMat mat; int obj; };
struct HostTri {
  v3 v0, v1, v2, norm;
  double cond = INFINITY;
  m33 ax, tuv;
  float tu0 = 0, tv0 = 0;
  int tex = -1;
  HostMat mat;
  int obj;
};
struct HostLight { v3 origin; float radius; float r, g, b, power; };
struct HostPlane { v3 pos, norm; HostMat mat; int obj; };

struct rfx_scene {
  col diff, env;
  float diff_power;
  float half_tile_w, half_tile_h;
  int skybox = -1;
  int tri_mates = 1;
  std::vector<HostSphere> spheres;
  std::vector<HostTri> tris;
  std::vector<HostPlane> planes;
  std::vector<int> obj_kind, obj_idx;
  std::vector<HostLight> lights;
  std::vector<HostTexture> textures;
};

static void default_half_tiles(rfx_scene *s)
{
  s->half_tile_w = 1.0f / 8.0f - kFltEpsilon;
  s->half_tile_h = 1.0f / 6.0f - kFltEpsilon;
}

extern "C" rfx_scene *rfx_scene_create(float dr, float dg, float db, float dp)
{
  rfx_scene *s = new rfx_scene();
  s->diff = mkc(dr, dg, db);
  s->diff_power = dp;
  s->env = cscale(s->diff, dp);
  default_half_tiles(s);
  return s;
}

extern "C" void rfx_scene_destroy(rfx_scene *s) { delete s; }

static HostMat make_mat(int type, const float rgb[3], float refl, float transp)
{
  HostMat m;
  m.dielectric = type == RFX_DIELECTRIC;
  m.r = rgb[0]; m.g = rgb[1]; m.b = rgb[2];
  m.refl = clampf(refl, 0.0f, 1.0f);
  m.transp = clampf(transp, 0.0f, 1.0f);
  return m;
}

extern "C" int rfx_scene_add_sphere(rfx_scene *s, const float c[3], float radius, int type, const float rgb[3],
                                    float refl, float transp)
{
  if (!s || !c || !rgb || (type != RFX_METAL && type != RFX_DIELECTRIC)) return fail(RFX_ERR_ARG, "add_sphere: bad args");
  if (radius <= kVerySmall) radius = kVerySmall;
  HostSphere sp;
  sp.center = mk(c[0], c[1], c[2]);
  sp.radius = radius;
  sp.sq_radius = radius * radius;
  sp.mat = make_mat(type, rgb, refl, transp);
  sp.obj = (int)s->obj_kind.size();
  s->obj_kind.push_back(0);
  s->obj_idx.push_back((int)s->spheres.size());
  s->spheres.push_back(sp);
  return sp.obj;
}

extern "C" int rfx_scene_add_triangle(rfx_scene *s, const float a[3], const float b[3], const float c[3], int type,
                                      const float rgb[3], float refl, float transp)
{
  if (!s || !a || !b || !c || !rgb || (type != RFX_METAL && type != RFX_DIELECTRIC))
    return fail(RFX_ERR_ARG, "add_triangle: bad args");
  HostTri t;
  const v3 v0 = mk(a[0], a[1], a[2]), v1 = mk(b[0], b[1], b[2]), v2 = mk(c[0], c[1], c[2]);
  t.v0 = v0;
  t.mat = make_mat(type, rgb, refl, transp);
  t.norm = normalized(cross(sub(v1, v0), sub(v2, v0)));
  const m33 basis = from_cols(sub(v2, v0), sub(v1, v0), neg(t.norm));
  t.ax = inverted(basis);
  t.v1 = v1;
  t.v2 = v2;
  {
    const float *a = &basis.m11, *b = &t.ax.m11;
    double na = 0.0, nb = 0.0;
    for (int k = 0; k < 9; ++k) { na += (double)a[k] * a[k]; nb += (double)b[k] * b[k]; }
    const float det = basis.m11 * (basis.m22 * basis.m33 - basis.m32 * basis.m23) +
                      basis.m21 * (basis.m32 * basis.m13 - basis.m12 * basis.m33) +
                      basis.m31 * (basis.m12 * basis.m23 - basis.m13 * basis.m22);
    t.cond = fabsf(det) > kVerySmall ? sqrt(na * nb) : INFINITY;
  }
  memset(&t.tuv, 0, sizeof(t.tuv));
  t.obj = (int)s->obj_kind.size();
  s->obj_kind.push_back(1);
  s->obj_idx.push_back((int)s->tris.size());
  s->tris.push_back(t);
  return t.obj;
}
// ... 451 lines not shown
{
  double lo[3] = {INFINITY, INFINITY, INFINITY}, hi[3] = {-INFINITY, -INFINITY, -INFINITY};
  for (const HostTri &t : tris)
  {
    if (!(t.cond < 300.0)) continue;
    for (const v3 &q : {t.v0, t.v1, t.v2})
    {
      const double c[3] = {q.x, q.y, q.z};
      for (int k = 0; k < 3; ++k) { lo[k] = fmin(lo[k], c[k]); hi[k] = fmax(hi[k], c[k]); }
    }
  }
  for (int k = 0; k < 3; ++k) ref[k] = lo[k] <= hi[k] ? (double)(float)(0.5 * (lo[k] + hi[k])) : 0.0;
}

extern "C" int rfx_scene_tri_bvh_dump(const rfx_scene *s, int32_t counts[5], float *boxes, int32_t *children,
                                      int32_t *leaf_ids, int32_t *residual)
{
  if (!s || !counts) return fail(RFX_ERR_ARG, "tri_bvh_dump: bad args");
  for (int k = 0; k < 5; ++k) counts[k] = 0;
  counts[3] = RFX_TRI_BVH_LEAF;
  if (s->spheres.size() <= 32 && s->tris.size() <= 32) return 0;
  TriTree T;
  double ref[3];
  tri_ref_point(s->tris, ref);
  if (!build_tri_tree(s->tris, ref, false, T)) return 0;
  counts[0] = (int32_t)T.nodes.size();
  counts[1] = (int32_t)T.leaves();
  counts[2] = (int32_t)T.resid.size();
  counts[4] = T.depth;
  for (size_t i = 0; i < T.nodes.size(); ++i)
  {
    const BvhNode &n = T.nodes[i];
    if (boxes)
      for (int c = 0; c < 2; ++c)
      {
        float *b = boxes + 12 * i + 6 * c;
        b[0] = n.lx[c]; b[1] = n.ly[c]; b[2] = n.lz[c]; b[3] = n.hx[c]; b[4] = n.hy[c]; b[5] = n.hz[c];
      }
    if (children) { children[2 * i] = n.child[0]; children[2 * i + 1] = n.child[1]; }
  }
  if (leaf_ids) std::copy(T.order.begin(), T.order.end(), leaf_ids);
  if (residual) std::copy(T.resid.begin(), T.resid.end(), residual);
  return 1;
}

static std::vector<int32_t> tri_mate_leaders(const std::vector<HostTri> &tris, bool on)
{
  std::vector<int32_t> leader(tris.size());
  std::map<std::array<uint32_t, 6>, int32_t> first;
  for (size_t i = 0; i < tris.size(); ++i)
  {
    const HostTri &t = tris[i];
    leader[i] = (int32_t)i;
    const float row[3] = {t.ax.m31, t.ax.m32, t.ax.m33}, v0[3] = {t.v0.x, t.v0.y, t.v0.z};
    bool finite = on;
    std::array<uint32_t, 6> key{};
    for (int a = 0; a < 3; ++a)
    {
      finite = finite && std::isfinite(row[a]) && std::isfinite(v0[a]);
      memcpy(&key[a], &row[a], 4);
      if (row[a] != 0.0f) memcpy(&key[3 + a], &v0[a], 4);
    }
    if (finite) leader[i] = first.emplace(key, (int32_t)i).first->second;
  }
  return leader;
}

extern "C" int rfx_scene_set_tri_mates(rfx_scene *s, int on)
{
  if (!s || on < 0 || on > 1) return fail(RFX_ERR_ARG, "scene_set_tri_mates: 0 or 1");
  s->tri_mates = on;
  return RFX_OK;
}

extern "C" int rfx_scene_tri_mates(const rfx_scene *s, int32_t *leader, float *plane)
{
  if (!s) return fail(RFX_ERR_ARG, "scene_tri_mates: null scene");
  const std::vector<int32_t> l = tri_mate_leaders(s->tris, s->tri_mates != 0);
  if (leader) std::copy(l.begin(), l.end(), leader);
  if (plane)
    for (const HostTri &t : s->tris)
      for (float f : {t.v0.x, t.v0.y, t.v0.z, t.ax.m31, t.ax.m32, t.ax.m33}) *plane++ = f;
  return (int)l.size();
}

static OrderBox order_box_of(const rfx_scene &s)
{
  float lo[3] = {INFINITY, INFINITY, INFINITY}, hi[3] = {-INFINITY, -INFINITY, -INFINITY};
  const auto take = [&](int a, float l, float h) {
    if (l < lo[a]) lo[a] = l;
    if (h > hi[a]) hi[a] = h;
  };
  for (size_t k = 0; k < s.obj_kind.size(); ++k)
  {
    if (s.obj_kind[k] == 0)
    {
      const HostSphere &h = s.spheres[s.obj_idx[k]];
      const float c[3] = {h.center.x, h.center.y, h.center.z};
      for (int a = 0; a < 3; ++a) take(a, c[a] - h.radius, c[a] + h.radius);
    }
    else if (s.obj_kind[k] == 1)
    {
      const HostTri &t = s.tris[s.obj_idx[k]];
      for (const v3 *v : {&t.v0, &t.v1, &t.v2})
      {
        take(0, v->x, v->x);
        take(1, v->y, v->y);
        take(2, v->z, v->z);
      }
    }
  }
  OrderBox b{};
  for (int a = 0; a < 3; ++a)
  {
    const bool ok = hi[a] > lo[a] && std::isfinite(lo[a]) && std::isfinite(hi[a]);
    b.scale[a] = ok ? (float)(1u << RFX_ORDER_CELL_BITS) / (hi[a] - lo[a]) : 0.0f;
    b.lo[a] = std::isfinite(lo[a]) ? lo[a] : 0.0f;
  }
  return b;
}

SceneBuild::SceneBuild(const rfx_scene &scene, int tri_accel)
{
  const rfx_scene *s = &scene;
  order_box = order_box_of(scene);
  const size_t nsph = s->spheres.size();
  std::vector<uint32_t> order(nsph);
  for (size_t i = 0; i < nsph; ++i) order[i] = (uint32_t)i;
  if (nsph > 32) spatial_order(order, 0, nsph, s->spheres);

  for (uint32_t oi : order)
  {
    const HostSphere &hs = s->spheres[oi];
    sg.push_back({hs.center.x, hs.center.y, hs.center.z, hs.sq_radius});
    sm.push_back({hs.mat.r, hs.mat.g, hs.mat.b, hs.mat.refl});
    si.push_back(hs.obj);
    si.push_back(hs.mat.dielectric);
  }
  const size_t npair_dev = sg.size() > 32 ? ((sg.size() + 1) / 2 + RFX_BVH_LEAF_PAIRS - 1) / RFX_BVH_LEAF_PAIRS *
                                                RFX_BVH_LEAF_PAIRS
                                          : (sg.size() + 1) / 2;
  sp.assign(npair_dev, SpherePair{});
  for (size_t i = 0; i < 2 * sp.size(); ++i)
  {
    SpherePair &p = sp[i / 2];
    const int l = (int)(i & 1);
    const bool real = i < sg.size();
    p.cx[l] = real ? sg[i].cx : 0.0f;
    p.cy[l] = real ? sg[i].cy : 0.0f;
    p.cz[l] = real ? sg[i].cz : 0.0f;
    p.r2[l] = real ? sg[i].sq_radius : -INFINITY;
  }
  for (const HostTri &t : s->tris)
  {
    TriGeo g{};
    g.v0x = t.v0.x; g.v0y = t.v0.y; g.v0z = t.v0.z;
    g.a11 = t.ax.m11; g.a12 = t.ax.m12; g.a13 = t.ax.m13;
    g.a21 = t.ax.m21; g.a22 = t.ax.m22; g.a23 = t.ax.m23;
    g.a31 = t.ax.m31; g.a32 = t.ax.m32; g.a33 = t.ax.m33;
    tg.push_back(g);
    TriShade h{};
    h.nx = t.norm.x; h.ny = t.norm.y; h.nz = t.norm.z;
    h.tu0 = t.tu0; h.tv0 = t.tv0;
    h.t11 = t.tuv.m11; h.t12 = t.tuv.m12; h.t21 = t.tuv.m21; h.t22 = t.tuv.m22;
    h.tex = t.tex; h.dielectric = t.mat.dielectric; h.obj = t.obj;
    ts.push_back(h);
// ... 80 lines not shown
        };
        double bc[3], ca[3];
        cross(Bv, Cv, bc);
        cross(Cv, A, ca);
        const double det = A[0] * bc[0] + A[1] * bc[1] + A[2] * bc[2];
        if (fabs(det) > 0.0)
        {
          const double gu[3] = {bc[0] / det, bc[1] / det, bc[2] / det}, gv[3] = {ca[0] / det, ca[1] / det, ca[2] / det};
          q.gux = (float)gu[0]; q.guy = (float)gu[1]; q.guz = (float)gu[2];
          q.gvx = (float)gv[0]; q.gvy = (float)gv[1]; q.gvz = (float)gv[2];
          q.nu = (float)(sqrt(gu[0] * gu[0] + gu[1] * gu[1] + gu[2] * gu[2]) * 1.001);
          q.nv = (float)(sqrt(gv[0] * gv[0] + gv[1] * gv[1] + gv[2] * gv[2]) * 1.001);
          const double s0 = gu[0] + gv[0], s1 = gu[1] + gv[1], s2 = gu[2] + gv[2];
          q.nuv = (float)(sqrt(s0 * s0 + s1 * s1 + s2 * s2) * 1.001);
        }
      }
      ct[i] = q;
    }
  }
  int bvh_depth = 0;
  double bvh_ref[3] = {0.0, 0.0, 0.0};
  if (nsph > 32)
  {
    const size_t npairs = ((nsph + 1) / 2 + RFX_BVH_LEAF_PAIRS - 1) / RFX_BVH_LEAF_PAIRS;
    constexpr size_t kLeafSph = 2 * RFX_BVH_LEAF_PAIRS;
    std::vector<PairBox> box(npairs);
    for (size_t j = 0; j < npairs; ++j)
    {
      PairBox &b = box[j];
      for (int k = 0; k < 3; ++k) { b.lo[k] = INFINITY; b.hi[k] = -INFINITY; }
      for (size_t q = kLeafSph * j; q < std::min(nsph, kLeafSph * j + kLeafSph); ++q)
      {
        const double c[3] = {bd[q].x, bd[q].y, bd[q].z}, rr = bd[q].r;
        for (int k = 0; k < 3; ++k) { b.lo[k] = fmin(b.lo[k], c[k] - rr); b.hi[k] = fmax(b.hi[k], c[k] + rr); }
      }
      for (int k = 0; k < 3; ++k) b.c[k] = 0.5 * (b.lo[k] + b.hi[k]);
    }
    std::vector<uint32_t> pairs(npairs);
    for (size_t j = 0; j < npairs; ++j) pairs[j] = (uint32_t)j;
    for (int k = 0; k < 3; ++k)
    {
      double lo = INFINITY, hi = -INFINITY;
      for (const PairBox &pb : box) { lo = fmin(lo, pb.lo[k]); hi = fmax(hi, pb.hi[k]); }
      bvh_ref[k] = (double)(float)(0.5 * (lo + hi));
    }
    build_pair_bvh(bvh, pairs, 0, npairs, box, bvh_ref, 0, bvh_depth);
    if (bvh_depth > kBvhStack) { bvh.clear(); bvh_depth = 0; }
    if (bvh.size() > 32767 || npairs > 32768) { bvh.clear(); bvh_depth = 0; }
  }
  const bool want_tri = RFX_TRI_BVH && !small &&
                        (tri_accel >= 1 || (tri_accel < 0 && s->tris.size() >= (size_t)RFX_TRI_BVH_AUTO_MIN));
  if (want_tri)
  {
    if (nsph <= 32) tri_ref_point(s->tris, bvh_ref);
    if (build_tri_tree(s->tris, bvh_ref, true, tt))
    {
      tleaf.assign(tt.order.size(), TriGeo{});
      for (size_t q = 0; q < tt.order.size(); ++q)
      {
        const int32_t i = tt.order[q];
        if (i < 0) continue;
        tleaf[q] = tg[i];
        const int32_t obj = s->tris[i].obj;
        memcpy(&tleaf[q].pad[0], &i, 4);
        memcpy(&tleaf[q].pad[1], &obj, 4);
      }
    }
  }
  for (const HostPlane &p : s->planes)
  {
    pg.push_back({p.pos.x, p.pos.y, p.pos.z, p.norm.x, p.norm.y, p.norm.z, p.obj, p.mat.dielectric});
    pm.push_back({p.mat.r, p.mat.g, p.mat.b, p.mat.refl});
  }
  loc.assign(s->obj_kind.size(), 0);
  {
    std::vector<int32_t> sph_dev(nsph);
    for (size_t di = 0; di < nsph; ++di) sph_dev[order[di]] = (int32_t)di;
    for (size_t o = 0; o < loc.size(); ++o)
    {
      const int kind = s->obj_kind[o], idx = s->obj_idx[o];
      loc[o] = kind << 28 | (kind == 0 ? sph_dev[idx] : idx);
    }
  }
  for (const HostLight &l : s->lights) lr.push_back({l.origin.x, l.origin.y, l.origin.z, l.radius, l.r, l.g, l.b, l.power});
  for (const HostTexture &t : s->textures)
  {
    const bool empty = t.texels.empty();
    tr.push_back({(uint32_t)pool.size(), empty ? 0u : t.w, empty ? 0u : t.h, 0});
    pool.insert(pool.end(), t.texels.begin(), t.texels.end());
  }
  d.n_tri_resid = (int32_t)tt.resid.size();
  d.n_tri_bvh = (int32_t)tt.nodes.size();
  d.tri_bvh_depth = tt.depth;
  accel.tri_nodes = d.n_tri_bvh;
  accel.tri_depth = tt.depth;
  accel.tri_leaf_size = RFX_TRI_BVH_LEAF;
  accel.tri_in_leaves = tt.nodes.empty() ? 0 : (int32_t)(s->tris.size() - tt.resid.size());
  accel.tri_residual = d.n_tri_resid;
  accel.sph_nodes = (int32_t)bvh.size();
  accel.sph_depth = bvh_depth;
  d.tri_bvh_narrow = !tt.nodes.empty() && (tri_accel == 2 || s->tris.size() >= (size_t)RFX_TRI_BVH_NARROW_MIN);
  accel.narrow_tri_bvh = d.tri_bvh_narrow;
  {
    float mt_max = 0.0f;
    for (const BvhNode &n : bvh) mt_max = fmaxf(mt_max, fmaxf(n.mt[0], n.mt[1]));
    const float mstep = mt_max > 0.0f ? mt_max / 65000.0f : 1.0f;
    aux.assign(2 * bvh.size(), 0u);
    for (size_t i = 0; i < bvh.size(); ++i)
    {
      const BvhNode &n = bvh[i];
      uint32_t q[2];
      for (int c = 0; c < 2; ++c) q[c] = (uint32_t)std::min(65535.0, ceil((double)n.mt[c] / mstep) + 1.0);
      aux[2 * i] = ((uint32_t)(uint16_t)(int16_t)n.child[0]) | ((uint32_t)(uint16_t)(int16_t)n.child[1] << 16);
      aux[2 * i + 1] = q[0] | q[1] << 16;
    }
    d.bvh_mstep = mstep;
    d.n_bvh = (int32_t)bvh.size();
  }
  d.n_sph = (int32_t)sg.size();
  d.n_tri = (int32_t)tg.size();
  d.n_light = (int32_t)lr.size();
  d.n_chunk = (int32_t)cb.size();
  d.n_pln = (int32_t)pg.size();
  d.n_tex = (int32_t)tr.size();
  d.bvh_depth = bvh_depth;
  d.bvh_rx = (float)bvh_ref[0]; d.bvh_ry = (float)bvh_ref[1]; d.bvh_rz = (float)bvh_ref[2];
  if (!bvh.empty())
  {
    const BvhNode &root = bvh[0];
    const float lo[3] = {fminf(root.lx[0], root.lx[1]), fminf(root.ly[0], root.ly[1]), fminf(root.lz[0], root.lz[1])};
    const float hi[3] = {fmaxf(root.hx[0], root.hx[1]), fmaxf(root.hy[0], root.hy[1]), fmaxf(root.hz[0], root.hz[1])};
    float s[3];
    for (int k = 0; k < 3; ++k) s[k] = hi[k] > lo[k] ? 8.0f / (hi[k] - lo[k]) : 0.0f;
    d.key_lx = lo[0]; d.key_ly = lo[1]; d.key_lz = lo[2];
    d.key_sx = s[0]; d.key_sy = s[1]; d.key_sz = s[2];
  }
  d.n_obj = (int32_t)loc.size();
  d.cull_valid = cull_valid;
  d.skybox_tex = s->skybox;
  const col amb = cscale(s->diff, s->diff_power);
  d.amb_r = amb.r; d.amb_g = amb.g; d.amb_b = amb.b;
  d.env_r = s->env.r; d.env_g = s->env.g; d.env_b = s->env.b;
  d.half_tile_w = s->half_tile_w;
  d.half_tile_h = s->half_tile_h;
}
```

reflaxman_amd/csrc/rfx_trace.h:

```cpp
#pragma once
#include <hip/hip_runtime.h>

#include "rfx_math.h"
#include "rfx_launch.h"
#include "rfx_types.h"
#include "rfx_shade_inputs.h"
#include "rfx_bounce.h"

#pragma clang fp contract(off)

namespace rfx {

template <bool STATS>
__device__ __forceinline__ void flush_counters(const FrameParams &P, Cnt &cnt)
{
  if constexpr (STATS)
  {
#pragma unroll
    for (int k = 0; k < C_COUNT; ++k)
    {
      unsigned long long v = cnt.c[k];
#pragma unroll
      for (int off = 32; off > 0; off >>= 1) v += __shfl_xor(v, off, 64);
      if ((threadIdx.x & 63) == 0 && v) atomicAdd(&P.counters[k], v);
// ... 37 lines not shown

__device__ __forceinline__ v3 rd_from_state(uint32_t s)
{
  const uint32_t s1 = lcg_step(s), s2 = lcg_step(s1), s3 = lcg_step(s2);
  return mk(rand_component_dev(lcg_out(s1)), rand_component_dev(lcg_out(s2)), rand_component_dev(lcg_out(s3)));
}

__device__ __forceinline__ v3 load_rd(const FrameParams &P, uint64_t i) { return rd_from_state(P.rd_state[i]); }

#ifdef RFX_DEBUG_WAVES
constexpr uint32_t kWaveTimeMax = 1u << 18;
constexpr uint32_t kBounceTimeBase = 1u << 17;
static __device__ unsigned long long g_wave_time[2 * kWaveTimeMax];
__device__ __forceinline__ uint64_t realtime64()
{
  uint64_t c;
  asm volatile("s_memrealtime %0\n\ts_waitcnt lgkmcnt(0)" : "=s"(c));
  return c;
}
#define RFX_WAVE_T0() const uint64_t wave_t0_ = realtime64()
#define RFX_WAVE_T1(tile)                                                                  \
  do {                                                                                      \
    const uint64_t t1_ = realtime64();                                                     \
    if (__lane_id() == 0 && (tile) < kWaveTimeMax)                                         \
    {                                                                                       \
      g_wave_time[2 * (tile)] = wave_t0_;                                                   \
      g_wave_time[2 * (tile) + 1] = t1_;                                                    \
    }                                                                                       \
  } while (0)
#else
constexpr uint32_t kBounceTimeBase = 0;
#define RFX_WAVE_T0() \
  do {                \
  } while (0)
#define RFX_WAVE_T1(tile) \
  do {                    \
  } while (0)
#endif

__device__ __forceinline__ uint32_t clock32()
{
  uint64_t c;
  asm("s_memtime %0\n\ts_waitcnt lgkmcnt(0)" : "=s"(c));
  return (uint32_t)c;
}


__device__ __forceinline__ void store_wave_tile(const FrameParams &P, uint32_t x0, uint32_t row0, col out,
                                                uint32_t lane, uint32_t wave)
{
  uint32_t *s = s_out[wave];
  s[3 * lane] = __float_as_uint(out.r);
  s[3 * lane + 1] = __float_as_uint(out.g);
  s[3 * lane + 2] = __float_as_uint(out.b);
  s[192 + lane] = argb(out);
  __builtin_amdgcn_wave_barrier();
  const bool rgb = lane < 48;
  const uint32_t k = rgb ? lane : lane - 48;
  const uint32_t r = rgb ? k / 6u : k >> 1, c = rgb ? k % 6u : k & 1u;
  const uint4 v = *reinterpret_cast<const uint4 *>(s + (rgb ? r * 24u + 4u * c : 192u + r * 8u + 4u * c));
  const size_t pix = (size_t)(row0 + r) * P.W + x0;
  uint32_t *dst = rgb ? reinterpret_cast<uint32_t *>(P.img) + pix * 3 + 4u * c : P.argb + pix + 4u * c;
  if (rgb || P.argb) *reinterpret_cast<uint4 *>(dst) = v;
}

enum TraceMode { kModeSsaa = 0, kModeBlock = 1, kModePlain = 2, kModeSsaaLanes = 3, kModeSsaaChunks = 4 };
__host__ __device__ constexpr uint32_t ss_lane_block(int ss)
{
  return ss == 1 ? 8u : ss == 2 ? 4u : ss == 4 ? 2u : ss >= 8 ? 1u : 0u;
}

#ifndef RFX_WAVES_PER_EU_LARGE
#define RFX_WAVES_PER_EU_LARGE RFX_WAVES_PER_EU
#endif
template <bool STATS, int MODE, int CFG>
__global__ __launch_bounds__(kWgThreads) __attribute__((amdgpu_waves_per_eu(
    (CFG & kCfgSmall) ? RFX_WAVES_PER_EU : RFX_WAVES_PER_EU_LARGE))) void trace_kernel(DevScene S, FrameParams P)
{
  static_assert(kKernargSig<decltype(&trace_kernel<STATS, MODE, CFG>)>, "launder_scene / kernarg_params layout");
  constexpr bool CULL = (CFG & kCfgCull) != 0, MANYL = (CFG & kCfgManyLights) != 0, SMALL = (CFG & kCfgSmall) != 0;
  constexpr bool PLANES = (CFG & kCfgPlanes) != 0, PARK = MODE == kModePlain && !STATS && (CFG & kCfgPark) != 0;
  constexpr bool ONEL = (CFG & kCfgOneLight) != 0;
  constexpr bool TBVH = (CFG & kCfgTriBvh) != 0;
  RFX_WAVE_T0();
  __shared__ float lut[256];
  for (uint32_t i = threadIdx.x; i < 256; i += kWgThreads) lut[i] = (float)i / 255.0f;
  stage_powf_tables();
  if constexpr (SMALL) stage_small_scene(S);
  RFX_PROF_INIT();
  __shared__ uint32_t s_clk0;
  if (P.tile_cost && threadIdx.x == 0) s_clk0 = clock32();
  __syncthreads();
  Cnt cnt;
  if constexpr (STATS)
  {
#pragma unroll
    for (int k = 0; k < C_COUNT; ++k) cnt.c[k] = 0;
  }
  const uint32_t lane = threadIdx.x & 63u, wave = threadIdx.x >> 6;
  const uint32_t wv = __builtin_amdgcn_readfirstlane(wave), wid = blockIdx.y * gridDim.x + blockIdx.x;
  const uint32_t w8 = kTileWavesX * gridDim.x;
  const uint32_t t8 = P.tile_order ? P.tile_order[kWgWaves * wid + wv]
                                   : (blockIdx.y * kTileWavesY + wv / kTileWavesX) * w8 + blockIdx.x * kTileWavesX + wv % kTileWavesX;
  const uint32_t gx = (t8 % w8) * 8u + (lane & 7u), gy = (t8 / w8) * 8u + (lane >> 3);
  if (lane == 0) s_tile8[wv] = t8;
  m33 view;
  view.m11 = P.v11; view.m12 = P.v12; view.m13 = P.v13;
  view.m21 = P.v21; view.m22 = P.v22; view.m23 = P.v23;
  view.m31 = P.v31; view.m32 = P.v32; view.m33 = P.v33;
  const v3 eye = mk(P.eye_x, P.eye_y, P.eye_z);

  if constexpr (MODE == kModeSsaaLanes || MODE == kModeSsaaChunks)
  {
    constexpr bool CHUNKS = MODE == kModeSsaaChunks;
    const uint32_t ss = (uint32_t)P.ss, ss2 = ss * ss, bw = CHUNKS ? 1u : ss_lane_block(P.ss);
    const uint32_t nchunk = CHUNKS ? (ss2 + 63) / 64 : 1;
    float *sm = reinterpret_cast<float *>(s_out[wv]);
    for (uint32_t chunk = 0; chunk < nchunk; ++chunk)
    {
      uint32_t lane = threadIdx.x & 63u;
      if constexpr (CHUNKS) asm volatile("" : "+v"(lane));
#ifdef RFX_LAUNDER_PARAMS
      const FrameParams &P = kernarg_params<CHUNKS>();
#endif
      const uint32_t q = bw == 1 ? 0 : lane / ss2, kk = bw == 1 ? 64 * chunk + lane : lane - q * ss2;
      const uint32_t sx = kk / ss, sy = kk - sx * ss;
      const uint32_t lx = (t8 % w8) * bw + q % bw, ly = (t8 / w8) * bw + q / bw;
      const uint32_t x = lx;
      const uint32_t y = P.nranks > 1 ? strip_row_to_y(ly, P) : ly + P.row0;
      const uint64_t p = (uint64_t)y * P.W + x;
      const bool valid = lx < P.W && ly < P.grid_rows && p >= P.p_begin && p < P.p_end && kk < ss2;
      const uint64_t pr = p - P.p_begin;
      float rndx = 0.0f, rndy = 0.0f;
      if (P.additive && valid)
      {
        const uint32_t s1 = lcg_jump(P.jitter_seed, 2 * pr + 1);
        rndx = (float)lcg_out(s1) / (float)0x7FFF;
        rndy = (float)lcg_out(lcg_step(s1)) / (float)0x7FFF;
      }
      const float ssf = (float)(int)ss;
      const float ox = sx ? (float)(int)sx / ssf : 0.0f, oy = sy ? (float)(int)sy / ssf : 0.0f;
      const float rx = (float)x - P.wh, ry = (float)y - P.hh;
      const v3 ray = mmul(view, mk(rx + ox + rndx, ry + oy + rndy, P.rz));
      v3 rd = mk(0.0f, 0.0f, 0.0f);
      if (valid) rd = load_rd(P, pr * (uint64_t)ss2 + kk);
      const uint64_t *pm = RFX_PRIM_LANES && SMALL && CULL && !STATS && P.prim_mask
                               ? P.prim_mask + (size_t)kPrimStride * t8 : nullptr;
      const col c = trace<STATS, CULL, MANYL, SMALL, PLANES, ONEL, TBVH>(S, eye, ray, P.depth, rd, lut, cnt, valid, pm,
                                                                  P.prim_shadow != 0);
      {
#ifdef RFX_LAUNDER_PARAMS
        const FrameParams &P = kernarg_params();
#endif
        const uint32_t t8e = ((volatile uint32_t *)s_tile8)[wv];
        uint32_t le = lane;
        asm volatile("" : "+v"(le));
        const uint32_t ss = (uint32_t)P.ss, ss2 = ss * ss, bw = CHUNKS ? 1u : ss_lane_block(P.ss);
        const uint32_t q = bw == 1 ? 0 : le / ss2, kk = bw == 1 ? 64 * chunk + le : le - q * ss2;
        const uint32_t lx = (t8e % w8) * bw + q % bw, ly = (t8e / w8) * bw + q / bw;
        const uint32_t x = lx;
        const uint32_t y = P.nranks > 1 ? strip_row_to_y(ly, P) : ly + P.row0;
        const uint64_t p = (uint64_t)y * P.W + x;
        const bool pvalid = lx < P.W && ly < P.grid_rows && p >= P.p_begin && p < P.p_end;
        sm[3 * le] = c.r;
        sm[3 * le + 1] = c.g;
        sm[3 * le + 2] = c.b;
        __builtin_amdgcn_wave_barrier();
        const uint32_t first = bw == 1 ? 64 * chunk : 0;
#if RFX_SSAA_CHANNEL_SUM
        if (ss2 >= 3)
        {
          const uint32_t lead = bw == 1 ? 0u : le - kk, ch = le - lead;
          const uint32_t n = min(ss2 - first, bw == 1 ? 64u : ss2);
          const bool last = first + n >= ss2;
          if (pvalid && ch < 3)
          {
            float fc = first ? sm[192 + ch] : 0.0f;
#pragma unroll 8
            for (uint32_t j = 0; j < n; ++j) fc = fc + sm[3 * (lead + j) + ch];
            if (!last)
              sm[192 + ch] = fc;
            else
            {
              const float sq = (float)(int)ss2;
              if (fabsf(sq) > kVerySmall) fc = fc / sq;
              const size_t o = (size_t)(P.nranks > 1 ? ly : y) * P.W + x;
              float *d = P.img + o * 3;
              if (P.accumulate) fc = d[ch] + fc;
              d[ch] = fc;
              sm[3 * lead + ch] = fc;
            }
          }
          __builtin_amdgcn_wave_barrier();
          if (last && pvalid && ch == 0 && P.argb)
            P.argb[(size_t)(P.nranks > 1 ? ly : y) * P.W + x] = argb(mkc(sm[3 * lead], sm[3 * lead + 1], sm[3 * lead + 2]));
        }
        else
#endif
        if (pvalid && (bw == 1 ? le == 0 : kk == 0))
        {
          col fin = first ? mkc(sm[192], sm[193], sm[194]) : mkc(0.0f, 0.0f, 0.0f);
          const uint32_t n = min(ss2 - first, bw == 1 ? 64u : ss2);
          for (uint32_t j = 0; j < n; ++j)
            fin = cadd(fin, mkc(sm[3 * (le + j)], sm[3 * (le + j) + 1], sm[3 * (le + j) + 2]));
          if (first + n < ss2)
          {
            sm[192] = fin.r;
            sm[193] = fin.g;
            sm[194] = fin.b;
          }
          else
          {
            const float sq = (float)(int)ss2;
            if (fabsf(sq) > kVerySmall) fin = mkc(fin.r / sq, fin.g / sq, fin.b / sq);
            const size_t o = (size_t)(P.nranks > 1 ? ly : y) * P.W + x;
            float *d = P.img + o * 3;
            if (P.accumulate) fin = mkc(d[0] + fin.r, d[1] + fin.g, d[2] + fin.b);
            d[0] = fin.r; d[1] = fin.g; d[2] = fin.b;
            if (P.argb) P.argb[o] = argb(fin);
          }
        }
        __builtin_amdgcn_wave_barrier();
        if (chunk + 1 == nchunk)
        {
          if (P.tile_cost && __lane_id() == 0) P.tile_cost[t8e] = clock32() - s_clk0;
          RFX_WAVE_T1(t8e);
        }
      }
    }
  }
  else if constexpr (MODE == kModeBlock)
  {
    const uint32_t n = (uint32_t)(-P.ss);
    const uint32_t bw = (P.W + n - 1) / n, bh = (P.H + n - 1) / n;
    const uint32_t cx = gx, cy = gy + P.row0;
    const uint32_t x = cx * n, y = cy * n;
    const uint64_t p = (uint64_t)y * P.W + x;
    const bool valid = gy < P.grid_rows && cx < bw && cy < bh && p >= P.p_begin && p < P.p_end;
    const v3 ray = mmul(view, mk((float)x - P.wh, (float)y - P.hh, P.rz));
    v3 rd = mk(0.0f, 0.0f, 0.0f);
    if (valid) rd = load_rd(P, (uint64_t)cy * bw + cx - P.trace_base);
    const col c = trace<STATS, CULL, MANYL, SMALL, PLANES, ONEL, TBVH>(S, eye, ray, P.depth, rd, lut, cnt, valid);
    if (valid)
    {
      const uint32_t ex = min(P.W, x + n), ey = min(P.H, y + n);
      const uint32_t a = argb(c);
      for (uint32_t qy = y; qy < ey; ++qy)
        for (uint32_t qx = x; qx < ex; ++qx)
        {
          float *d = P.img + ((size_t)qy * P.W + qx) * 3;
          d[0] = c.r; d[1] = c.g; d[2] = c.b;
          if (P.argb) P.argb[(size_t)qy * P.W + qx] = a;
        }
    }
  }
  else
  {
    const uint32_t x = gx;
    const uint32_t y = P.nranks > 1 ? strip_row_to_y(gy, P) : gy + P.row0;
    const uint64_t p = (uint64_t)y * P.W + x;
    const bool valid = gx < P.W && gy < P.grid_rows && p >= P.p_begin && p < P.p_end;
    const uint64_t pr = p - P.p_begin;
    const float rx = (float)x - P.wh, ry = (float)y - P.hh;
    col out;
    bool parked = false;
    if constexpr (MODE == kModePlain)
    {
      const v3 ray = mmul(view, mk(rx + 0.0f + 0.0f, ry + 0.0f + 0.0f, P.rz));
      v3 rd = mk(0.0f, 0.0f, 0.0f);
      if (valid) rd = load_rd(P, pr);
      const ParkTile park{P.park_after, P.queue, P.queue_count, P, wv, w8};
      const uint64_t *pm_tile = SMALL && CULL && !STATS && P.prim_mask ? P.prim_mask + (size_t)kPrimStride * t8 : nullptr;
      const col c = trace_from<STATS, CULL, MANYL, SMALL, PLANES, PARK, ParkTile, ONEL, TBVH>(S, eye, ray, mkc(1.0f, 1.0f, 1.0f),
                                                                  mkc(0.0f, 0.0f, 0.0f), 0, P.depth, rd, lut, cnt,
                                                                  valid, park, parked, pm_tile);
      out = cadd(mkc(0.0f, 0.0f, 0.0f), c);
    }
    else
    {
      float rndx = 0.0f, rndy = 0.0f;
      if (P.additive && valid)
      {
        const uint32_t s1 = lcg_jump(P.jitter_seed, 2 * pr + 1);
        rndx = (float)lcg_out(s1) / (float)0x7FFF;
        rndy = (float)lcg_out(lcg_step(s1)) / (float)0x7FFF;
      }
      const int ss = P.ss;
      const float ssf = (float)ss;
      col fin = mkc(0.0f, 0.0f, 0.0f);
      for (int sx = 0; sx < ss; ++sx)
        for (int sy = 0; sy < ss; ++sy)
        {
          const float ox = sx ? (float)sx / ssf : 0.0f, oy = sy ? (float)sy / ssf : 0.0f;
          v3 ray = mk(rx + ox + rndx, ry + oy + rndy, P.rz);
          ray = mmul(view, ray);
          v3 rd = mk(0.0f, 0.0f, 0.0f);
          if (valid) rd = load_rd(P, pr * (uint64_t)(ss * ss) + (uint64_t)(sx * ss + sy));
          const uint64_t *pm = RFX_PRIM_SSAA && SMALL && CULL && !STATS && P.prim_mask
                                   ? P.prim_mask + (size_t)kPrimStride * t8 : nullptr;
          fin = cadd(fin, trace<STATS, CULL, MANYL, SMALL, PLANES, false, TBVH>(S, eye, ray, P.depth, rd, lut, cnt, valid, pm,
                                                                   P.prim_shadow != 0));
        }
      if (ss != 1)
      {
        const float sq = (float)(ss * ss);
        if (fabsf(sq) > kVerySmall) fin = mkc(fin.r / sq, fin.g / sq, fin.b / sq);
      }
      out = fin;
    }
#ifdef RFX_LAUNDER_PARAMS
    const FrameParams &P = kernarg_params();
#endif
    const uint32_t t8e = ((volatile uint32_t *)s_tile8)[wv];
    uint32_t le = lane;
    asm volatile("" : "+v"(le));
    const uint32_t x0e = (t8e % w8) * 8u, row0e = (t8e / w8) * 8u + (P.nranks > 1 ? 0u : P.row0);
    const uint32_t xe = x0e + (le & 7u), rowe = row0e + (le >> 3), wslot = wv;
    if (MODE == kModeSsaa && P.accumulate && valid)
    {
      const float *d = P.img + ((size_t)rowe * P.W + xe) * 3;
      out = mkc(d[0] + out.r, d[1] + out.g, d[2] + out.b);
    }
    const bool staged = (P.W & 3u) == 0 &&
                        ((reinterpret_cast<uintptr_t>(P.img) | reinterpret_cast<uintptr_t>(P.argb)) & 15u) == 0 &&
                        __builtin_amdgcn_ballot_w64(valid && !parked) == ~0ull;
    if (staged)
      store_wave_tile(P, x0e, row0e, out, le, wslot);
    else if (valid && !parked)
    {
      const size_t o = (size_t)rowe * P.W + xe;
      float *d = P.img + o * 3;
      d[0] = out.r; d[1] = out.g; d[2] = out.b;
      if (P.argb) P.argb[o] = argb(out);
    }
    if (P.tile_cost && __lane_id() == 0)
      P.tile_cost[(P.nranks > 1 ? rowe : rowe - P.row0) / 8u * P.tiles_x + xe / 8u] = clock32() - s_clk0;
    RFX_WAVE_T1(t8e);
  }
  flush_counters<STATS>(P, cnt);
  RFX_PROF_FLUSH();

}

template <bool STATS, int MODE, int CFG>
inline void launch_one(dim3 grid, const DevScene &S, const FrameParams &P, hipStream_t st)
{
  if constexpr (!STATS || !(CFG & kCfgCull))
    hipLaunchKernelGGL((trace_kernel<STATS, MODE, CFG>), grid, dim3(kWgThreads), 0, st, S, P);
}

template <bool STATS, int MODE>
inline void launch_cfg(int cfg, dim3 grid, const DevScene &S, const FrameParams &P, hipStream_t st)
{
#if RFX_TRI_BVH
  if (cfg & kCfgTriBvh)
  {
    if constexpr (!STATS)
      switch (cfg & ~kCfgTriBvh)
      {
        case 1: launch_one<STATS, MODE, 1 | kCfgTriBvh>(grid, S, P, st); return;
        case 3: launch_one<STATS, MODE, 3 | kCfgTriBvh>(grid, S, P, st); return;
        case 9: launch_one<STATS, MODE, 9 | kCfgTriBvh>(grid, S, P, st); return;
        case 11: launch_one<STATS, MODE, 11 | kCfgTriBvh>(grid, S, P, st); return;
        case 1 | kCfgOneLight: launch_one<STATS, MODE, 1 | kCfgOneLight | kCfgTriBvh>(grid, S, P, st); return;
        case 9 | kCfgOneLight: launch_one<STATS, MODE, 9 | kCfgOneLight | kCfgTriBvh>(grid, S, P, st); return;
      }
    cfg &= ~kCfgTriBvh;
  }
#endif
  if (cfg & kCfgOneLight)
  {
    switch (cfg & ~kCfgOneLight)
    {
      case 1: launch_one<STATS, MODE, 1 | kCfgOneLight>(grid, S, P, st); return;
      case 5: launch_one<STATS, MODE, 5 | kCfgOneLight>(grid, S, P, st); return;
      case 9: launch_one<STATS, MODE, 9 | kCfgOneLight>(grid, S, P, st); return;
      case 13: launch_one<STATS, MODE, 13 | kCfgOneLight>(grid, S, P, st); return;
      default: cfg &= ~kCfgOneLight;
    }
  }
  switch (cfg)
  {
    case 0: launch_one<STATS, MODE, 0>(grid, S, P, st); break;
    case 1: launch_one<STATS, MODE, 1>(grid, S, P, st); break;
    case 2: launch_one<STATS, MODE, 2>(grid, S, P, st); break;
    case 3: launch_one<STATS, MODE, 3>(grid, S, P, st); break;
    case 4: launch_one<STATS, MODE, 4>(grid, S, P, st); break;
    case 5: launch_one<STATS, MODE, 5>(grid, S, P, st); break;
    case 6: launch_one<STATS, MODE, 6>(grid, S, P, st); break;
    case 7: launch_one<STATS, MODE, 7>(grid, S, P, st); break;
    case 8: launch_one<STATS, MODE, 8>(grid, S, P, st); break;
    case 9: launch_one<STATS, MODE, 9>(grid, S, P, st); break;
    case 10: launch_one<STATS, MODE, 10>(grid, S, P, st); break;
    case 11: launch_one<STATS, MODE, 11>(grid, S, P, st); break;
    case 12: launch_one<STATS, MODE, 12>(grid, S, P, st); break;
    case 13: launch_one<STATS, MODE, 13>(grid, S, P, st); break;
    case 14: launch_one<STATS, MODE, 14>(grid, S, P, st); break;
    case 15: launch_one<STATS, MODE, 15>(grid, S, P, st); break;
  }
}

}
```

reflaxman_amd/csrc/rfx_trace_plain_park.hip:

```cpp
#include "rfx_trace.h"
#include "rfx_parked.h"

#include <atomic>

namespace rfx {

constexpr int kLdsLimitDevices = 64;

template <int CFG>
static void launch_park_one(dim3 grid, const DevScene &S, const FrameParams &P, hipStream_t st)
{
  hipLaunchKernelGGL((trace_kernel<false, kModePlain, CFG | kCfgPark>), grid, dim3(kWgThreads), 0, st, S, P);
}

void launch_trace_plain_park(int cfg, dim3 grid, const DevScene &S, const FrameParams &P, hipStream_t st)
{
  switch (cfg & ~kCfgPark)
  {
#if RFX_TRI_BVH
    case 1 | kCfgTriBvh: launch_park_one<1 | kCfgTriBvh>(grid, S, P, st); break;
    case 3 | kCfgTriBvh: launch_park_one<3 | kCfgTriBvh>(grid, S, P, st); break;
    case 9 | kCfgTriBvh: launch_park_one<9 | kCfgTriBvh>(grid, S, P, st); break;
    case 11 | kCfgTriBvh: launch_park_one<11 | kCfgTriBvh>(grid, S, P, st); break;
    case 1 | kCfgOneLight | kCfgTriBvh: launch_park_one<1 | kCfgOneLight | kCfgTriBvh>(grid, S, P, st); break;
    case 9 | kCfgOneLight | kCfgTriBvh: launch_park_one<9 | kCfgOneLight | kCfgTriBvh>(grid, S, P, st); break;
#endif
    case 1 | kCfgOneLight: launch_park_one<1 | kCfgOneLight>(grid, S, P, st); break;
    case 5 | kCfgOneLight: launch_park_one<5 | kCfgOneLight>(grid, S, P, st); break;
    case 1: launch_park_one<1>(grid, S, P, st); break;
    case 3: launch_park_one<3>(grid, S, P, st); break;
    case 5: launch_park_one<5>(grid, S, P, st); break;
    case 7: launch_park_one<7>(grid, S, P, st); break;
    case 9: launch_park_one<9>(grid, S, P, st); break;
    case 11: launch_park_one<11>(grid, S, P, st); break;
    case 13: launch_park_one<13>(grid, S, P, st); break;
    case 15: launch_park_one<15>(grid, S, P, st); break;
    default:
      if (cfg & kCfgOneLight) launch_trace_plain_park(cfg & ~kCfgOneLight, grid, S, P, st);
      break;
  }
}

template <int CFG>
static void launch_bounce_one(dim3 grid, const DevScene &S, const FrameParams &P, hipStream_t st)
{
  hipLaunchKernelGGL((bounce_kernel<CFG>), grid, dim3(kWgThreads), 0, st, S, P);
}

template <int CFG>
static hipError_t launch_bounce_lds_one(uint32_t groups, const DevScene &S, const FrameParams &P, hipStream_t st)
{
  static std::atomic<int> limit_set[kLdsLimitDevices];
  int dev = 0;
  const bool cached = hipGetDevice(&dev) == hipSuccess && dev >= 0 && dev < kLdsLimitDevices;
  int state = cached ? limit_set[dev].load(std::memory_order_relaxed) : 0;
  if (state == 0)
  {
    state = hipFuncSetAttribute(reinterpret_cast<const void *>(&bounce_kernel_lds<CFG>),
                                hipFuncAttributeMaxDynamicSharedMemorySize, 160 * 1024 - 4096) == hipSuccess ? 1 : 2;
    if (cached) limit_set[dev].store(state, std::memory_order_relaxed);
  }
  if (state != 1) return hipErrorInvalidValue;
  hipLaunchKernelGGL((bounce_kernel_lds<CFG>), dim3(groups), dim3(kLdsBvhThreads), lds_bvh_bytes(S.n_bvh), st, S, P);
  return hipGetLastError();
}

hipError_t launch_bounce_lds(int cfg, uint32_t groups, const DevScene &S, const FrameParams &P, hipStream_t st)
{
  switch (cfg)
  {
#if RFX_TRI_BVH
    case 1 | kCfgTriBvh: return launch_bounce_lds_one<1 | kCfgTriBvh>(groups, S, P, st);
    case 3 | kCfgTriBvh: return launch_bounce_lds_one<3 | kCfgTriBvh>(groups, S, P, st);
    case 9 | kCfgTriBvh: return launch_bounce_lds_one<9 | kCfgTriBvh>(groups, S, P, st);
    case 11 | kCfgTriBvh: return launch_bounce_lds_one<11 | kCfgTriBvh>(groups, S, P, st);
    case 1 | kCfgOneLight | kCfgTriBvh: return launch_bounce_lds_one<1 | kCfgOneLight | kCfgTriBvh>(groups, S, P, st);
    case 9 | kCfgOneLight | kCfgTriBvh: return launch_bounce_lds_one<9 | kCfgOneLight | kCfgTriBvh>(groups, S, P, st);
#endif
    case 1 | kCfgOneLight: return launch_bounce_lds_one<1 | kCfgOneLight>(groups, S, P, st);
    case 9 | kCfgOneLight: return launch_bounce_lds_one<9 | kCfgOneLight>(groups, S, P, st);
    case 1: return launch_bounce_lds_one<1>(groups, S, P, st);
    case 3: return launch_bounce_lds_one<3>(groups, S, P, st);
    case 9: return launch_bounce_lds_one<9>(groups, S, P, st);
    case 11: return launch_bounce_lds_one<11>(groups, S, P, st);
    default:
      return (cfg & kCfgOneLight) ? launch_bounce_lds(cfg & ~kCfgOneLight, groups, S, P, st) : hipErrorInvalidValue;
  }
}

void launch_bounce(int cfg, dim3 grid, const DevScene &S, const FrameParams &P, hipStream_t st)
{
  switch (cfg)
  {
#if RFX_TRI_BVH
    case 1 | kCfgTriBvh: launch_bounce_one<1 | kCfgTriBvh>(grid, S, P, st); break;
    case 3 | kCfgTriBvh: launch_bounce_one<3 | kCfgTriBvh>(grid, S, P, st); break;
    case 9 | kCfgTriBvh: launch_bounce_one<9 | kCfgTriBvh>(grid, S, P, st); break;
    case 11 | kCfgTriBvh: launch_bounce_one<11 | kCfgTriBvh>(grid, S, P, st); break;
    case 1 | kCfgOneLight | kCfgTriBvh: launch_bounce_one<1 | kCfgOneLight | kCfgTriBvh>(grid, S, P, st); break;
    case 9 | kCfgOneLight | kCfgTriBvh: launch_bounce_one<9 | kCfgOneLight | kCfgTriBvh>(grid, S, P, st); break;
#endif
    case 1 | kCfgOneLight: launch_bounce_one<1 | kCfgOneLight>(grid, S, P, st); break;
    case 5 | kCfgOneLight: launch_bounce_one<5 | kCfgOneLight>(grid, S, P, st); break;
    case 1: launch_bounce_one<1>(grid, S, P, st); break;
    case 3: launch_bounce_one<3>(grid, S, P, st); break;
    case 5: launch_bounce_one<5>(grid, S, P, st); break;
    case 7: launch_bounce_one<7>(grid, S, P, st); break;
    case 9: launch_bounce_one<9>(grid, S, P, st); break;
    case 11: launch_bounce_one<11>(grid, S, P, st); break;
    case 13: launch_bounce_one<13>(grid, S, P, st); break;
    case 15: launch_bounce_one<15>(grid, S, P, st); break;
    default:
      if (cfg & kCfgOneLight) launch_bounce(cfg & ~kCfgOneLight, grid, S, P, st);
      break;
  }
}

}

#ifdef RFX_DEBUG_WAVES
extern "C" int rfx_debug_wave_time_read_park(unsigned long long *out, int n)
// ... 8 lines not shown
```

reflaxman_amd/csrc/rfx_types.h:

```cpp
#pragma once
#include "rfx_config.h"

#include <stddef.h>
#include <stdint.h>

namespace rfx {

enum Counter {
  C_RAYS = 0, C_SEGMENTS,
  C_SPH_TESTS, C_SPH_B, C_SPH_D, C_SPH_T,
  C_TRI_TESTS, C_TRI_Z, C_TRI_S, C_TRI_T, C_TRI_IN, C_TRI_D,
  C_HIT_SPH, C_HIT_TRI,
  C_SH_SPH_TESTS, C_SH_SPH_B, C_SH_SPH_D, C_SH_SPH_T,
  C_SH_TRI_TESTS, C_SH_TRI_Z, C_SH_TRI_S, C_SH_TRI_T, C_SH_TRI_IN,
  C_L_EVAL, C_L_FACING, C_L_LIT, C_L_SPEC, C_L_POW,
  C_DIELECTRIC, C_METAL, C_CONTINUE, C_SKY,
  C_TEX_BILINEAR, C_TEX_CHECKER, C_TEX_OTHER,
  C_PLN_TESTS, C_PLN_T, C_HIT_PLN, C_SH_PLN_TESTS, C_SH_PLN_T,
  C_COUNT
};

struct alignas(16) SphereGeo { float cx, cy, cz, sq_radius; };
struct alignas(32) SpherePair { float cx[2], cy[2], cz[2], r2[2]; };
struct alignas(16) MatRec { float r, g, b, refl; };
struct alignas(16) TriGeo {
  float v0x, v0y, v0z, a31, a32, a33;
  float a11, a21, a12, a22, a13, a23;
  float pad[4];
};
struct alignas(16) TriShade {
  float nx, ny, nz, tu0;
  float t11, t12, t21, t22;
  float tv0; int32_t tex; int32_t dielectric; int32_t obj;
};
struct alignas(16) Bound { float x, y, z, r; };
struct alignas(16) CullRec { float x, y, z, r, nx, ny, nz, d; };
struct alignas(16) CullTri { float v0x, v0y, v0z, nu, gux, guy, guz, nv, gvx, gvy, gvz, nuv; };
constexpr int kBvhStack = 16;
struct alignas(16) BvhNode { float lx[2], ly[2], lz[2], hx[2], hy[2], hz[2]; int32_t child[2]; float mt[2]; };
struct alignas(16) PlaneGeo { float px, py, pz, nx, ny, nz; int32_t obj, dielectric; };
struct alignas(16) LightRec { float ox, oy, oz, radius, r, g, b, power; };
struct alignas(16) TexRec { uint32_t offset, w, h, pad; };

struct DevScene {
  const SphereGeo *sph_geo;
  const SpherePair *sph_pair;
  const MatRec *sph_mat;
  const int32_t *sph_info;
  const TriGeo *tri_geo;
  const TriShade *tri_shade;
  const MatRec *tri_mat;
  const LightRec *lights;
  const TexRec *texs;
  const uint32_t *texels;
  const Bound *bound;
  const Bound *chunk_bound;
  const BvhNode *bvh;
  const CullRec *cull_small;
  const CullTri *cull_tri;
  const PlaneGeo *pln_geo;
  const MatRec *pln_mat;
  const int32_t *obj_loc;
  uint64_t cull_valid;
  int32_t n_sph, n_tri, n_light, skybox_tex;
  int32_t n_pln, n_obj, n_tex;
  int32_t bvh_depth;
  float bvh_rx, bvh_ry, bvh_rz;
  float key_lx, key_ly, key_lz;
  float key_sx, key_sy, key_sz;
  int32_t n_chunk;
  const uint32_t *bvh_aux;
  float bvh_mstep;
  int32_t n_bvh;
  float amb_r, amb_g, amb_b;
  float env_r, env_g, env_b;
  float half_tile_w, half_tile_h;
  const BvhNode *tri_bvh;
  const TriGeo *tri_leaf;
  const int32_t *tri_resid;
  int32_t n_tri_resid;
  int32_t n_tri_bvh;
  int32_t tri_bvh_depth;
  int32_t tri_bvh_narrow;
};

constexpr int kLdsBvhWaves = 16, kLdsBvhStackSlots = 16;
constexpr size_t lds_bvh_bytes(int n_bvh)
{
  return (size_t)n_bvh * 56 + sizeof(int16_t) * kLdsBvhStackSlots * 64 * kLdsBvhWaves + 4 * 64 * kLdsBvhWaves;
}
constexpr bool lds_bvh_fits(int n_bvh) { return n_bvh > 0 && lds_bvh_bytes(n_bvh) + 4096 <= 160 * 1024; }

constexpr uint32_t kQueueBuckets = 4096;
struct alignas(16) QRay {
  float ox, oy, oz, dx;
  float dy, dz, mr, mg;
  float mb, pr, pg, pb;
  uint32_t trace, out, refl, pad;
};

struct FrameParams {
  float eye_x, eye_y, eye_z;
  float v11, v12, v13, v21, v22, v23, v31, v32, v33;
  float rz, wh, hh;
  uint32_t W, H;
  int32_t depth, ss;
  int32_t accumulate;
  int32_t additive;
  uint32_t jitter_seed;
  uint32_t row_block, rank, nranks;
  uint32_t grid_rows;
  uint32_t row0;
  uint64_t p_begin, p_end;
  uint64_t trace_base;
  float *img;
  uint32_t *argb;
  const uint32_t *rd_state;
  unsigned long long *counters;
  const uint32_t *tile_order;
  uint32_t *tile_cost;
  uint32_t tiles_x;
  QRay *queue;
  uint32_t *queue_count, *queue_next;
  int32_t park_after;
  uint32_t *queue_key;
  const uint32_t *queue_order;
  const uint64_t *prim_mask;
  int32_t prim_shadow;
};

struct HitParams {
  const float *rays;
  const int32_t *skip;
  uint64_t n;
  uint32_t W;
  int32_t *object;
  float *distance, *point, *normal, *reflected, *colour;
  uint8_t *occluded;
};

constexpr int kPrimLights = 4, kPrimStride = 1 + kPrimLights;
constexpr int kCfgCull = 1, kCfgManyLights = 2, kCfgSmall = 4, kCfgPlanes = 8, kCfgPark = 16, kCfgOneLight = 32;
constexpr int kCfgTriBvh = 64;

}
```

reflaxman_amd/render.py:

```python
from __future__ import annotations

import ctypes as C
import os
from typing import List, Optional, Sequence

import numpy as np

from . import _lib
from ._lib import DIELECTRIC, METAL, check, farr

DEFAULT_SPHERE_SEED = 1350490027
DEFAULT_JITTER_SEED = 424238335


class Vector3:
    __slots__ = ("x", "y", "z")

    def __init__(self, x=0.0, y=0.0, z=0.0):
        self.x, self.y, self.z = float(x), float(y), float(z)

    def __iter__(self):
        return iter((self.x, self.y, self.z))

    def __repr__(self):
# ... 60 lines not shown


class Sphere:
    def __init__(self, scene: "Scene", obj: int):
        self.scene, self.obj = scene, obj


class Plane:

    def __init__(self, scene: "Scene", obj: int):
        self.scene, self.obj = scene, obj


class OmniLight:
    def __init__(self, scene: "Scene", index: int):
        self.scene, self.index = scene, index


class Scene:

    def __init__(self, diffLightColor: Color = Color(0, 0, 0), diffLightPower: float = 0.0):
        L = _lib.load()
        self._h = C.c_void_p(L.rfx_scene_create(*Color(*diffLightColor), float(diffLightPower)))
        if not self._h:
            raise _lib.RfxError("rfx_scene_create failed")
        self._version = 0
        self._keep = []

    def __del__(self):
        h = getattr(self, "_h", None)
        if h and _lib._lib is not None:
            _lib._lib.rfx_scene_destroy(h)
            self._h = None

    def addSphere(self, center: Vector3, radius: float, material: Material) -> Sphere:
        obj = check(_lib.load().rfx_scene_add_sphere(self._h, farr(Vector3(*center)), float(radius), material.type,
                                                     farr(material.color), material.reflectivity, material.transparency),
                    "Scene.addSphere")
        self._version += 1
        return Sphere(self, obj)

    def addTriangle(self, v1: Vector3, v2: Vector3, v3: Vector3, material: Material) -> Triangle:
        obj = check(_lib.load().rfx_scene_add_triangle(self._h, farr(Vector3(*v1)), farr(Vector3(*v2)), farr(Vector3(*v3)),
                                                       material.type, farr(material.color), material.reflectivity,
                                                       material.transparency), "Scene.addTriangle")
        self._version += 1
        return Triangle(self, obj)

    def addMesh(self, vertices, indices, material: Material) -> List[Triangle]:
        v = np.ascontiguousarray(vertices, dtype=np.float32).reshape(-1, 3)
        i = np.ascontiguousarray(indices, dtype=np.uint32).reshape(-1, 3)
        first = check(_lib.load().rfx_scene_add_mesh(self._h, _lib.fptr(v), v.shape[0], _lib.u32ptr(i), i.shape[0],
                                                     material.type, farr(material.color), material.reflectivity,
                                                     material.transparency), "Scene.addMesh")
        self._version += 1
        return [Triangle(self, first + k) for k in range(i.shape[0])]

    def tri_bvh_dump(self):
        L = _lib.load()
        cnt = (C.c_int32 * 5)()
        if check(L.rfx_scene_tri_bvh_dump(self._h, cnt, None, None, None, None), "Scene.tri_bvh_dump") == 0:
            return None
        nodes, leaves, nres, leaf, depth = (int(x) for x in cnt)
        boxes = np.zeros((nodes, 2, 6), np.float32)
        children = np.zeros((nodes, 2), np.int32)
        ids = np.zeros((leaves, leaf), np.int32)
        res = np.zeros(nres, np.int32)
        i32 = lambda a: a.ctypes.data_as(_lib._i32p)
        check(L.rfx_scene_tri_bvh_dump(self._h, cnt, _lib.fptr(boxes), i32(children), i32(ids), i32(res)),
              "Scene.tri_bvh_dump")
        return {"nodes": nodes, "leaves": leaves, "leaf_size": leaf, "depth": depth, "boxes": boxes,
                "children": children, "leaf_ids": ids, "residual": res}

    def set_tri_mates(self, on: bool):
        check(_lib.load().rfx_scene_set_tri_mates(self._h, int(bool(on))), "Scene.set_tri_mates")
        self._version += 1

    def tri_mates(self, plane: bool = False):
        L = _lib.load()
        n = check(L.rfx_scene_tri_mates(self._h, None, None), "Scene.tri_mates")
        leader, rows = np.zeros(n, np.int32), np.zeros((n, 6), np.float32)
        check(L.rfx_scene_tri_mates(self._h, leader.ctypes.data_as(_lib._i32p), _lib.fptr(rows)), "Scene.tri_mates")
        return (leader, rows) if plane else leader

    def addPlane(self, pos: Vector3, norm: Vector3, material: Material) -> Plane:
        obj = check(_lib.load().rfx_scene_add_plane(self._h, farr(Vector3(*pos)), farr(Vector3(*norm)), material.type,
                                                    farr(material.color), material.reflectivity, material.transparency),
                    "Scene.addPlane")
        self._version += 1
        return Plane(self, obj)

    def addLight(self, origin: Vector3, radius: float, color: Color, power: float) -> OmniLight:
        idx = check(_lib.load().rfx_scene_add_light(self._h, farr(Vector3(*origin)), float(radius), farr(Color(*color)),
                                                    float(power)), "Scene.addLight")
        self._version += 1
        return OmniLight(self, idx)

    def addTexture(self, fileName: str) -> Texture:
        loaded = C.c_int(0)
        idx = check(_lib.load().rfx_scene_add_texture_file(self._h, os.fsencode(fileName), C.byref(loaded)),
                    "Scene.addTexture")
        self._version += 1
        return Texture(self, idx, bool(loaded.value))

    def addTextureArgb(self, argb: Optional[np.ndarray]) -> Texture:
        L = _lib.load()
        if argb is None:
            idx = check(L.rfx_scene_add_texture_argb(self._h, 0, 0, None), "Scene.addTextureArgb")
        else:
            a = np.ascontiguousarray(argb, dtype=np.uint32)
            idx = check(L.rfx_scene_add_texture_argb(self._h, a.shape[1], a.shape[0], _lib.u32ptr(a)), "Scene.addTextureArgb")
        self._version += 1
        return Texture(self, idx, argb is not None)

    def setSkyboxTexture(self, fileName: str) -> bool:
        ok = check(_lib.load().rfx_scene_set_skybox_file(self._h, os.fsencode(fileName)), "Scene.setSkyboxTexture")
        self._version += 1
        return bool(ok)

    def setSkyboxTextureArgb(self, argb: Optional[np.ndarray]) -> bool:
        L = _lib.load()
        if argb is None:
            ok = check(L.rfx_scene_set_skybox_argb(self._h, 0, 0, None), "Scene.setSkyboxTextureArgb")
        else:
            a = np.ascontiguousarray(argb, dtype=np.uint32)
            ok = check(L.rfx_scene_set_skybox_argb(self._h, a.shape[1], a.shape[0], _lib.u32ptr(a)), "Scene.setSkyboxTextureArgb")
        self._version += 1
        return bool(ok)

    def counts(self):
        v = [C.c_int() for _ in range(4)]
        check(_lib.load().rfx_scene_counts(self._h, *[C.byref(x) for x in v]), "Scene.counts")
        return tuple(x.value for x in v)


def build_scene(desc, texture_dir: Optional[str] = None) -> tuple:
    d = desc.diffuse
    s = Scene(Color(d[0], d[1], d[2]), d[3])
    files = {}
    if texture_dir is not None:
        path = desc.write(texture_dir)
        for line in open(path):
            parts = line.split()
            if parts and parts[0] in ("skybox", "texture"):
                files.setdefault(parts[0], []).append(
                    None if parts[1] == "-" else os.path.join(texture_dir, parts[1]))
    if desc.skybox is not None:
        if texture_dir is not None:
            s.setSkyboxTexture(files["skybox"][0] or "/nonexistent/absent.tga")
        else:
            s.setSkyboxTextureArgb(desc.skybox.argb)
    for (o, r, c, p) in desc.lights:
        s.addLight(Vector3(*o), r, Color(*c), p)
    if texture_dir is not None:
        texs = [s.addTexture(f or "/nonexistent/absent.tga") for f in files.get("texture", [])]
    else:
        texs = [s.addTextureArgb(t.argb) for t in desc.textures]
    handles = []
    for ob in desc.objects:
        mt, rgb, refl, tr = ob[-1]
        m = Material(mt, Color(*rgb), refl, tr)
        if ob[0] == "sphere":
            handles.append(s.addSphere(Vector3(*ob[1]), ob[2], m))
        elif ob[0] == "plane":
            handles.append(s.addPlane(Vector3(*ob[1]), Vector3(*ob[2]), m))
        else:
# ... 394 lines not shown
        check(_lib.load().rfx_renderer_set_tile_order(self._h, int(mode)), "set_tile_order")

    def set_prim_masks(self, mode: int):
        check(_lib.load().rfx_renderer_set_prim_masks(self._h, int(mode)), "set_prim_masks")

    def set_prim_exact(self, on: bool):
        check(_lib.load().rfx_renderer_set_prim_exact(self._h, int(bool(on))), "set_prim_exact")

    def prim_masks(self) -> np.ndarray:
        L = _lib.load()
        n = C.c_uint64()
        check(L.rfx_renderer_get_prim_masks(self._h, None, 0, C.byref(n)), "get_prim_masks")
        out = np.zeros(n.value, np.uint64)
        if n.value:
            check(L.rfx_renderer_get_prim_masks(self._h, _lib.u64ptr(out), n.value, C.byref(n)), "get_prim_masks")
        return out

    def set_regroup(self, park_after: int):
        check(_lib.load().rfx_renderer_set_regroup(self._h, int(park_after)), "set_regroup")

    def set_regroup_sort(self, on: bool):
        check(_lib.load().rfx_renderer_set_regroup_sort(self._h, int(bool(on))), "set_regroup_sort")

    def set_launch_traces(self, max_traces: int):
        check(_lib.load().rfx_renderer_set_launch_traces(self._h, int(max_traces)), "set_launch_traces")

    def bounce_form(self) -> int:
        return _lib.load().rfx_renderer_bounce_form(self._h)

    def set_rng_prepass(self, mode: int):
        check(_lib.load().rfx_renderer_set_rng_prepass(self._h, int(mode)), "set_rng_prepass")

    def prepass_form(self) -> int:
        return _lib.load().rfx_renderer_prepass_form(self._h)

    def kat_rng_seq_prefix(self) -> np.ndarray:
        out = np.zeros(_lib.load().rfx_rng_seq_blocks() + 1, np.uint32)
        check(_lib.load().rfx_kat_rng_seq_prefix(self._h, _lib.u32ptr(out)), "rfx_kat_rng_seq_prefix")
        return out

    def kat_rng_seq_legacy(self) -> np.ndarray:
        out = np.zeros(_lib.load().rfx_rng_seq_blocks(), np.uint32)
        check(_lib.load().rfx_kat_rng_seq_legacy(self._h, _lib.u32ptr(out)), "rfx_kat_rng_seq_legacy")
        return out

    def set_tri_accel(self, mode: int):
        check(_lib.load().rfx_renderer_set_tri_accel(self._h, int(mode)), "set_tri_accel")
        self._scene_key = None

    def accel_info(self) -> "_lib.AccelInfo":
        a = _lib.AccelInfo()
        check(_lib.load().rfx_renderer_accel_info(self._h, C.byref(a)), "accel_info")
        return a

    def set_timing(self, enable):
        check(_lib.load().rfx_renderer_set_timing(self._h, int(enable)), "set_timing")

    def get_timing(self):
        a, b, n = C.c_double(), C.c_double(), C.c_uint64()
        check(_lib.load().rfx_renderer_get_timing(self._h, C.byref(a), C.byref(b), C.byref(n)), "get_timing")
        return a.value, b.value, n.value

    def kat_objects(self, rays: np.ndarray, objects: np.ndarray) -> np.ndarray:
        rays = np.ascontiguousarray(rays, np.float32).reshape(-1, 6)
        objs = np.ascontiguousarray(objects, np.int32)
        out = np.zeros((rays.shape[0], 15), np.float32)
        check(_lib.load().rfx_kat_objects(self._h, _lib.fptr(rays), objs.ctypes.data_as(C.POINTER(C.c_int32)),
                                          rays.shape[0], _lib.fptr(out)), "rfx_kat_objects")
        return out

    def kat_texels(self, texture: int, inp: np.ndarray) -> np.ndarray:
        inp = np.ascontiguousarray(inp, np.float32)
        out = np.zeros((inp.shape[0], 3), np.float32)
        check(_lib.load().rfx_kat_texels(self._h, int(texture), _lib.fptr(inp), inp.shape[0], _lib.fptr(out)),
              "rfx_kat_texels")
        return out

    def kat_powf(self, xy: np.ndarray) -> np.ndarray:
        xy = np.ascontiguousarray(xy, np.float32)
        out = np.zeros(xy.shape[0], np.float32)
        check(_lib.load().rfx_kat_powf(self._h, _lib.fptr(xy), xy.shape[0], _lib.fptr(out)), "rfx_kat_powf")
        return out

    def kat_powf_cube(self):
        counts = (C.c_uint64 * 2)()
        check(_lib.load().rfx_kat_powf_cube(self._h, counts), "rfx_kat_powf_cube")
        return int(counts[0]), int(counts[1])

    def kat_argb(self, rgb: np.ndarray) -> np.ndarray:
        rgb = np.ascontiguousarray(rgb, np.float32)
        out = np.zeros(rgb.shape[0], np.uint32)
        check(_lib.load().rfx_kat_argb(self._h, _lib.fptr(rgb), rgb.shape[0], _lib.u32ptr(out)), "rfx_kat_argb")
        return out

    def rand_dirs(self, seed: int, n: int):
        out = np.zeros((n, 3), np.float32)
        after = C.c_uint32()
        check(_lib.load().rfx_rand_dirs(self._h, seed, n, _lib.fptr(out), C.byref(after)), "rfx_rand_dirs")
        return out, after.value


def make_frame(camera: Camera, W: int, H: int, reflect_num: int, sample_num: int = 1, additive: bool = False,
               additive_counter: int = 0, row_block: int = 0, rank: int = 0, nranks: int = 1,
               pixel_begin: int = 0, pixel_end: int = 0) -> _lib.Frame:
    f = _lib.Frame()
    f.eye[:] = list(camera.eye)
    f.view[:] = list(camera.view)
    f.fov = camera.fov
    f.width, f.height = W, H
    f.reflect_num, f.sample_num = reflect_num, sample_num
    f.additive, f.additive_counter = int(bool(additive)), additive_counter
    f.row_block, f.rank, f.nranks = row_block, rank, nranks
    f.pixel_begin, f.pixel_end = pixel_begin, pixel_end
    return f


class Render:

    def __init__(self, exePath: str = "", device: int = 0, sphere_seed: int = DEFAULT_SPHERE_SEED,
                 jitter_seed: int = DEFAULT_JITTER_SEED, load_default_scene: bool = True):
        self._r = Renderer(device, sphere_seed, jitter_seed)
        self.imageWidth = 0
        self.imageHeight = 0
        self.additiveCounter = 0
        self.inProgress = False
        self._curx = 0
        self._cury = 0
        self._d_img = None
        self._cap = 0
        self._host = None
        self._host_valid = False
        self.camera = Camera()
        self.scene = Scene()
        self._refl = 0
        self._ss = 0
        self._additive = False
        if load_default_scene:
            self.loadScene(exePath)

    def loadScene(self, exePath: str):
        from . import scenes
        sky = os.path.join(exePath, "./textures/skybox.tga")
        plane = os.path.join(exePath, "./textures/himiya.tga")
        self.camera = Camera(Vector3(*scenes.DEFAULT_CAMERA[0]), Vector3(*scenes.DEFAULT_CAMERA[1]), scenes.DEFAULT_CAMERA[2])
        self.scene = Scene(Color(0.95, 0.95, 1.0), 0.15)
        self.scene.setSkyboxTexture(sky)
        self.scene.addLight(Vector3(11.8e9, 4.26e9, 3.08e9), 3.48e8, Color(1.0, 1.0, 0.95), 0.85)
        for (c, r, mt, rgb, refl) in [
            ((-1.25, 1.5, -0.25), 1.5, METAL, (1.0, 1.0, 1.0), 1.0), ((0.15, 1.0, 1.75), 1.0, METAL, (1.0, 1.0, 1.0), 0.95),
            ((-3.0, 0.6, -3.0), 0.6, DIELECTRIC, (1.0, 1.0, 1.0), 0.0), ((-0.5, 0.5, -2.5), 0.5, DIELECTRIC, (0.5, 1.0, 0.15), 0.75),
            ((1.0, 0.4, -1.5), 0.4, DIELECTRIC, (0.0, 0.5, 1.0), 1.0), ((1.8, 0.4, 0.1), 0.4, METAL, (1.0, 0.65, 0.45), 1.0),
            ((1.7, 0.5, 1.9), 0.5, METAL, (1.0, 0.90, 0.60), 0.75), ((0.6, 0.6, 4.2), 0.6, METAL, (0.9, 0.9, 0.9), 0.0)]:
            self.scene.addSphere(Vector3(*c), r, Material(mt, Color(*rgb), refl, 0.0))
        tex = self.scene.addTexture(plane)
        tr1 = self.scene.addTriangle(Vector3(-14.0, 0.0, -10.0), Vector3(-14.0, 0.0, 10.0), Vector3(14.0, 0.0, -10.0),
                                     Material(DIELECTRIC, Color(1.0, 1.0, 1.0), 0.95, 0.0))
        tr1.setTexture(tex, 0.0, 0.0, 0.0, 1.0, 1.0, 0.0)
        tr2 = self.scene.addTriangle(Vector3(-14.0, 0.0, 10.0), Vector3(14.0, 0.0, 10.0), Vector3(14.0, 0.0, -10.0),
                                     Material(DIELECTRIC, Color(1.0, 1.0, 1.0), 0.95, 0.0))
        tr2.setTexture(tex, 0.0, 1.0, 1.0, 1.0, 1.0, 0.0)

    def setImageSize(self, width: int, height: int):
        if width <= 0 or height <= 0:
            return
        L = _lib.load()
        n = width * height * 3 * 4
# ... 130 lines not shown
```

Measured before the change: 13680 Mrays/s.

## Precompute far-light shading terms and use a fixed shadow cone for distant sun

For single-light small scenes whose geometry sits well inside the light's float-rounding neighbourhood, the host precomputes light direction, distance, specular offset and a shadow-cone angle, and stores them in an extended LightRec. Hit points near the origin reuse these terms instead of recomputing length, normalize and sqrt per shade. Shadow bundles use a fixed cone aligned with the light when the whole wave is near, instead of building one per wave. This adds a kernel variant, a bigger light record and an exact-equality validity condition that depends on scene extent.

```diff
diff --git a/include/rfx.h b/include/rfx.h
--- a/include/rfx.h
+++ b/include/rfx.h
@@ -52,6 +52,8 @@
                            int32_t *leaf_ids, int32_t *residual);
 int rfx_scene_set_tri_mates(rfx_scene *scene, int on);
 int rfx_scene_tri_mates(const rfx_scene *scene, int32_t *leader, float *plane);
+int rfx_scene_set_far_lights(rfx_scene *scene, int mode);
+int rfx_scene_far_light(const rfx_scene *scene, int light, float terms[8]);
 
 void rfx_camera_view(const float eye[3], const float at[3], float view[9]);
 float rfx_camera_rz(uint32_t width, float fov);
@@ -214,6 +216,7 @@
 
 int rfx_rand_dirs(rfx_renderer *r, uint32_t seed, uint64_t n, float *out3, uint32_t *seed_out);
 
+int rfx_kat_far_light(rfx_renderer *r, const float *points, uint64_t n, float *out);
 int rfx_kat_objects(rfx_renderer *r, const float *rays, const int32_t *objects, uint64_t n, float *out);
 int rfx_kat_texels(rfx_renderer *r, int texture, const float *in, uint64_t n, float *out);
 int rfx_kat_powf(rfx_renderer *r, const float *xy, uint64_t n, float *out);
diff --git a/reflaxman_amd/_lib.py b/reflaxman_amd/_lib.py
--- a/reflaxman_amd/_lib.py
+++ b/reflaxman_amd/_lib.py
@@ -59,6 +59,8 @@
     ("rfx_scene_tri_bvh_dump", C.c_int, [C.c_void_p, _i32p, _fp, _i32p, _i32p, _i32p]),
     ("rfx_scene_set_tri_mates", C.c_int, [C.c_void_p, C.c_int]),
     ("rfx_scene_tri_mates", C.c_int, [C.c_void_p, _i32p, _fp]),
+    ("rfx_scene_set_far_lights", C.c_int, [C.c_void_p, C.c_int]),
+    ("rfx_scene_far_light", C.c_int, [C.c_void_p, C.c_int, _fp]),
     ("rfx_scene_add_plane", C.c_int, [C.c_void_p, _fp, _fp, C.c_int, _fp, C.c_float, C.c_float]),
     ("rfx_scene_plane_count", C.c_int, [C.c_void_p]),
     ("rfx_triangle_set_texture", C.c_int, [C.c_void_p, C.c_int, C.c_int, _fp]),
@@ -159,6 +161,7 @@
     ("rfx_kat_objects", C.c_int, [C.c_void_p, _fp, C.POINTER(C.c_int32), C.c_uint64, _fp]),
     ("rfx_kat_texels", C.c_int, [C.c_void_p, C.c_int, _fp, C.c_uint64, _fp]),
     ("rfx_kat_powf", C.c_int, [C.c_void_p, _fp, C.c_uint64, _fp]),
+    ("rfx_kat_far_light", C.c_int, [C.c_void_p, _fp, C.c_uint64, _fp]),
     ("rfx_kat_argb", C.c_int, [C.c_void_p, _fp, C.c_uint64, _u32p]),
     ("rfx_kat_powf_cube", C.c_int, [C.c_void_p, C.POINTER(C.c_uint64)]),
     ("rfx_kat_div", C.c_int, [C.c_void_p, C.c_uint64, C.c_uint64, C.POINTER(C.c_uint64)]),
diff --git a/reflaxman_amd/csrc/rfx_bounce.h b/reflaxman_amd/csrc/rfx_bounce.h
--- a/reflaxman_amd/csrc/rfx_bounce.h
+++ b/reflaxman_amd/csrc/rfx_bounce.h
@@ -73,8 +73,21 @@
   return *(const FrameParams *)(const __attribute__((address_space(4))) FrameParams *)(p + kParamsOff);
 }
 
+__device__ __forceinline__ bool near_light(const LightRec &L, v3 d)
+{
+  return fabsf(d.x) < L.near && fabsf(d.y) < L.near && fabsf(d.z) < L.near;
+}
+
+__device__ __forceinline__ LightRec reread_light(const LightRec *l, uint64_t when)
+{
+  typedef const __attribute__((address_space(4))) LightRec *ConstLightPtr;
+  ConstLightPtr p = (ConstLightPtr)l;
+  asm("" : "+s"(p) : "s"(when));
+  return *(const LightRec *)p;
+}
+
 template <bool STATS, bool CULL, bool MANYL, bool SMALL, bool PLANES, bool PARK, class PK, bool ONEL = false,
-          bool TBVH = false>
+          bool TBVH = false, bool FARL = false>
 __device__ __forceinline__ col trace_from(const DevScene &RFX_SCENE_PARAM, v3 origin, v3 ray, col mulc, col pix, int refl,
                                           int depth, v3 rd, const float *lut, Cnt &cnt, bool valid, const PK &park,
                                           bool &parked, const uint64_t *pm_tile = nullptr, bool pm_shadow = true)
@@ -82,6 +95,9 @@
 #ifdef RFX_LAUNDER_SCENE
   const DevScene &S = S_in;
 #endif
+  static_assert(!FARL || (ONEL && SMALL && CULL && !MANYL && !STATS), "FARL: the small-scene one-light culling kernels");
+  constexpr bool FAR_SHADE = FARL && (RFX_FAR_LIGHT == 1 || RFX_FAR_LIGHT == 2);
+  constexpr bool FAR_CONE = FARL && (RFX_FAR_LIGHT == 1 || RFX_FAR_LIGHT == 3);
   bool seg0 = pm_tile != nullptr;
   parked = false;
   if (valid && refl == 0) RFX_CNT(C_RAYS);
@@ -190,7 +206,11 @@
                 om = pm_tile[1 + q];
               else
               {
-                const Bundle SB = make_bundle(drop, sray, facing);
+                Bundle SB;
+                bool far_cone = false;
+                if constexpr (FAR_CONE) far_cone = __ballot(facing && !near_light(L, drop)) == 0;
+                if (far_cone) SB = make_bundle_far(drop, L, facing);
+                else SB = make_bundle(drop, sray, facing);
                 if (SB.ok) om = cull_small(T.cull(), S.cull_valid, SB);
                 RFX_CULL_STAT(1, SB.ok, __ballot(facing), om, S.cull_valid);
               }
@@ -242,7 +262,43 @@
         {
           if (!((lit >> q) & 1u)) continue;
           RFX_CNT(C_L_LIT);
-          const LightRec L = S.lights[base + q];
+          const LightRec L = FAR_SHADE ? reread_light(S.lights + (base + q), __ballot(lit != 0)) : S.lights[base + q];
+          if constexpr (FAR_SHADE)
+          {
+            v3 dtl = mk(L.ox, L.oy, L.oz), ndl = mk(L.ndx, L.ndy, L.ndz);
+            float dlen = L.dlen, spec_add = L.spec_add;
+            bool spec = true;
+            if (!near_light(L, drop))
+            {
+              dtl = sub(dtl, drop);
+              dlen = len(dtl);
+              const float a2 = sqlen(dtl);
+              const float ang = (a2 > kVerySmall) ? 1.0f - qdiv(L.radius * L.radius, a2) : 0.0f;
+              spec = ang > 0;
+              if (spec)
+              {
+                ndl = normalized(dtl);
+                spec_add = 1.0f - sqrt_rn(ang);
+              }
+            }
+            float aa = dlen * normLen;
+            const float cosl = (aa > kVerySmall) ? qdiv(dot(dtl, norm), aa) : 0.0f;
+            const col lc = mkc(L.r, L.g, L.b);
+            if (L.power > kVerySmall) sumL = cadd(sumL, cscale(cscale(lc, cosl), L.power));
+            if (spec)
+            {
+              const v3 dlr = add(ndl, mul(rd, 1.0f - m.refl));
+              aa = len(dlr) * reflectLen;
+              float sc = (aa > kVerySmall) ? qdiv(dot(dlr, reflv), aa) : 0.0f;
+              sc = clampf(sc + spec_add, 0.0f, 1.0f);
+              if (sc > kVerySmall && L.radius > kVerySmall)
+              {
+                const float sp = powf_dev(sc, 1 + qdiv(3 * m.refl * dlen, L.radius)) * m.refl;
+                sumS = cadd(sumS, cscale(lc, sp));
+              }
+            }
+            continue;
+          }
           const v3 dtl = sub(mk(L.ox, L.oy, L.oz), drop);
           const float dlen = len(dtl);
           float aa = dlen * normLen;
@@ -350,12 +406,13 @@
 #endif
 }
 
-template <bool STATS, bool CULL, bool MANYL, bool SMALL, bool PLANES, bool ONEL = false, bool TBVH = false>
+template <bool STATS, bool CULL, bool MANYL, bool SMALL, bool PLANES, bool ONEL = false, bool TBVH = false,
+          bool FARL = false>
 __device__ __forceinline__ col trace(const DevScene &S, v3 origin, v3 ray, int depth, v3 rd, const float *lut,
                                      Cnt &cnt, bool valid, const uint64_t *pm_tile = nullptr, bool pm_shadow = true)
 {
   bool parked;
-  return trace_from<STATS, CULL, MANYL, SMALL, PLANES, false, Park, ONEL, TBVH>(S, origin, ray, mkc(1.0f, 1.0f, 1.0f), mkc(0.0f, 0.0f, 0.0f), 0,
+  return trace_from<STATS, CULL, MANYL, SMALL, PLANES, false, Park, ONEL, TBVH, FARL>(S, origin, ray, mkc(1.0f, 1.0f, 1.0f), mkc(0.0f, 0.0f, 0.0f), 0,
                                                        depth, rd, lut, cnt, valid, Park{0, nullptr, nullptr, 0, 0},
                                                        parked, pm_tile, pm_shadow);
 }
diff --git a/reflaxman_amd/csrc/rfx_bundle.h b/reflaxman_amd/csrc/rfx_bundle.h
--- a/reflaxman_amd/csrc/rfx_bundle.h
+++ b/reflaxman_amd/csrc/rfx_bundle.h
@@ -88,6 +88,23 @@
   B.cosa = 1.0f - devm - 4e-6f;
   B.sina = __builtin_amdgcn_sqrtf(fmaxf(1.0f - B.cosa * B.cosa, 0.0f) + 1e-7f) * 1.001f;
   B.ok = __ballot(bad) == 0 && B.cosa > 0.1f && B.rw <= 1.0e15f;
+  return B;
+}
+
+__device__ __forceinline__ Bundle make_bundle_far(v3 o, const LightRec &L, bool live)
+{
+  Bundle B;
+  const int ref = __ffsll((long long)__ballot(live)) - 1;
+  B.cx = lane_bcast(o.x, ref); B.cy = lane_bcast(o.y, ref); B.cz = lane_bcast(o.z, ref);
+  B.ax = L.ndx; B.ay = L.ndy; B.az = L.ndz;
+  const float ex = o.x - B.cx, ey = o.y - B.cy, ez = o.z - B.cz;
+  const float e2 = cdot(ex, ey, ez, ex, ey, ez);
+  const bool bad = live && !(e2 <= 1.0e30f);
+  const float e2m = wave_max_nonneg(live ? e2 : 0.0f);
+  B.rw = __builtin_amdgcn_sqrtf(e2m) * 1.0001f;
+  B.cosa = L.cone_cos;
+  B.sina = L.cone_sin;
+  B.ok = __ballot(bad) == 0 && B.rw <= 1.0e15f;
   return B;
 }
 
diff --git a/reflaxman_amd/csrc/rfx_config.h b/reflaxman_amd/csrc/rfx_config.h
--- a/reflaxman_amd/csrc/rfx_config.h
+++ b/reflaxman_amd/csrc/rfx_config.h
@@ -34,6 +34,9 @@
 #endif
 #ifndef RFX_TRI_MATES
 #define RFX_TRI_MATES 2
+#endif
+#ifndef RFX_FAR_LIGHT
+#define RFX_FAR_LIGHT 1
 #endif
 #ifndef RFX_CULL_FMA
 #define RFX_CULL_FMA 1
diff --git a/reflaxman_amd/csrc/rfx_kat.cpp b/reflaxman_amd/csrc/rfx_kat.cpp
--- a/reflaxman_amd/csrc/rfx_kat.cpp
+++ b/reflaxman_amd/csrc/rfx_kat.cpp
@@ -58,6 +58,13 @@
 {
   if (!r || (n && (!xy || !out))) return fail(RFX_ERR_ARG, "kat_powf: bad args");
   return kat_run(r, 2, 0, xy, (size_t)n * 2, nullptr, n, out, (size_t)n);
+}
+
+extern "C" int rfx_kat_far_light(rfx_renderer *r, const float *points, uint64_t n, float *out)
+{
+  if (!r || (n && (!points || !out))) return fail(RFX_ERR_ARG, "kat_far_light: bad args");
+  if (!r->has_scene || r->dev.n_light < 1) return fail(RFX_ERR_STATE, "kat_far_light: no scene with a light uploaded");
+  return kat_run(r, 4, 0, points, (size_t)n * 3, nullptr, n, out, (size_t)n * 8);
 }
 
 extern "C" int rfx_kat_argb(rfx_renderer *r, const float *rgb, uint64_t n, uint32_t *out)
diff --git a/reflaxman_amd/csrc/rfx_kernels.hip b/reflaxman_amd/csrc/rfx_kernels.hip
--- a/reflaxman_amd/csrc/rfx_kernels.hip
+++ b/reflaxman_amd/csrc/rfx_kernels.hip
@@ -927,6 +927,29 @@
     const float x = xy[2 * (size_t)i], y = xy[2 * (size_t)i + 1];
     out[i] = y == 3.0f ? powf3_dev(x) : powf_dev(x, y);
   }
+}
+
+__global__ __launch_bounds__(kKatThreads) void kat_far_light(DevScene S, const float *d, uint32_t n, float *out)
+{
+  const uint32_t i = blockIdx.x * kKatThreads + threadIdx.x;
+  if (i >= n) return;
+  const LightRec L = S.lights[0];
+  const v3 drop = mk(d[3 * (size_t)i], d[3 * (size_t)i + 1], d[3 * (size_t)i + 2]);
+  const v3 dtl = sub(mk(L.ox, L.oy, L.oz), drop);
+  const float dlen = len(dtl), aa = sqlen(dtl);
+  const float ang = (aa > kVerySmall) ? 1.0f - qdiv(L.radius * L.radius, aa) : 0.0f;
+  const v3 nd = normalized(dtl);
+  const float spec_add = ang > 0 ? 1.0f - sqrt_rn(ang) : 0.0f;
+  float v[8] = {dtl.x, dtl.y, dtl.z, dlen, nd.x, nd.y, nd.z, spec_add};
+  if (near_light(L, drop))
+  {
+    const float w[8] = {L.ox, L.oy, L.oz, L.dlen, L.ndx, L.ndy, L.ndz, L.spec_add};
+    bool same = ang > 0 && L.radius > kVerySmall;
+    for (int k = 0; k < 8; ++k) same = same && __float_as_uint(v[k]) == __float_as_uint(w[k]);
+    if (!same)
+      for (int k = 0; k < 8; ++k) v[k] = __builtin_nanf("");
+  }
+  for (int k = 0; k < 8; ++k) out[8 * (size_t)i + k] = v[k];
 }
 
 __global__ __launch_bounds__(kKatThreads) void kat_powf_cube(uint32_t first, uint32_t n, unsigned long long *counts)
@@ -1243,6 +1266,7 @@
     case 0: hipLaunchKernelGGL(kat_objects, kat_grid(n), dim3(kKatThreads), 0, st, S, (const float *)in, objs, n, (float *)out); break;
     case 1: hipLaunchKernelGGL(kat_texels, kat_grid(n), dim3(kKatThreads), 0, st, S, tex, (const float *)in, n, (float *)out); break;
     case 2: hipLaunchKernelGGL(kat_powf, kat_grid(n), dim3(kKatThreads), 0, st, (const float *)in, n, (float *)out); break;
+    case 4: hipLaunchKernelGGL(kat_far_light, kat_grid(n), dim3(kKatThreads), 0, st, S, (const float *)in, n, (float *)out); break;
     default: hipLaunchKernelGGL(kat_argb, kat_grid(n), dim3(kKatThreads), 0, st, (const float *)in, n, (uint32_t *)out); break;
   }
   return hipGetLastError();
@@ -1325,10 +1349,13 @@
   const int mode = trace_mode(P);
   const bool cull = !stats && !(RFX_NOCULL_MAX_TILES > 0 && S.n_sph <= 32 && S.n_tri <= 32 &&
                                 trace_tiles(P) <= (uint32_t)RFX_NOCULL_MAX_TILES);
-  const int cfg = (S.n_light > 32 ? kCfgManyLights : 0) | (cull ? kCfgCull : 0) |
-                  (S.n_sph <= 32 && S.n_tri <= 32 ? kCfgSmall : 0) | (S.n_pln > 0 ? kCfgPlanes : 0) |
-                  (S.n_light == 1 && !stats && RFX_ONE_LIGHT ? kCfgOneLight : 0) |
-                  (RFX_TRI_BVH && S.tri_bvh != nullptr && !stats ? kCfgTriBvh : 0);
+  int cfg = (S.n_light > 32 ? kCfgManyLights : 0) | (cull ? kCfgCull : 0) |
+            (S.n_sph <= 32 && S.n_tri <= 32 ? kCfgSmall : 0) | (S.n_pln > 0 ? kCfgPlanes : 0) |
+            (S.n_light == 1 && !stats && RFX_ONE_LIGHT ? kCfgOneLight : 0) |
+            (RFX_TRI_BVH && S.tri_bvh != nullptr && !stats ? kCfgTriBvh : 0);
+  const bool far_mode = mode == kModePlain || mode == kModeSsaaLanes || mode == kModeSsaaChunks;
+  if (RFX_FAR_LIGHT && S.far_light && far_mode && (cfg & ~kCfgPlanes) == (kCfgCull | kCfgSmall | kCfgOneLight))
+    cfg |= kCfgFarLight;
   launch_mode_cfg(stats, mode, cfg, grid, S, Pt, st);
   return hipGetLastError();
 }
diff --git a/reflaxman_amd/csrc/rfx_scene.cpp b/reflaxman_amd/csrc/rfx_scene.cpp
--- a/reflaxman_amd/csrc/rfx_scene.cpp
+++ b/reflaxman_amd/csrc/rfx_scene.cpp
@@ -54,6 +54,7 @@
   float half_tile_w, half_tile_h;
   int skybox = -1;
   int tri_mates = 1;
+  int far_lights = 1;
   std::vector<HostSphere> spheres;
   std::vector<HostTri> tris;
   std::vector<HostPlane> planes;
@@ -671,6 +672,69 @@
     for (const HostTri &t : s->tris)
       for (float f : {t.v0.x, t.v0.y, t.v0.z, t.ax.m31, t.ax.m32, t.ax.m33}) *plane++ = f;
   return (int)l.size();
+}
+
+static LightRec far_light_terms(const HostLight &l)
+{
+  LightRec rec{l.origin.x, l.origin.y, l.origin.z, l.radius, l.r, l.g, l.b, l.power, 0, 0, 0, 0, 0, 0, 0, 0};
+  const float c[3] = {l.origin.x, l.origin.y, l.origin.z};
+  float near = INFINITY;
+  for (int a = 0; a < 3; ++a)
+  {
+    if (!std::isfinite(c[a])) return rec;
+    const float m = fabsf(c[a]);
+    near = fminf(near, (m - nextafterf(m, 0.0f)) / 2);
+  }
+  if (!std::isfinite(l.radius) || !(near > 0.0f)) return rec;
+  const v3 dtl = l.origin;
+  const float aa = sqlen(dtl);
+  if (!std::isfinite(aa) || !(aa > kVerySmall)) return rec;
+  const float ang = 1.0f - qdiv(l.radius * l.radius, aa);
+  if (!(ang > 0) || !(l.radius > kVerySmall)) return rec;
+  const float dlen = len(dtl);
+  const float sb = fminf(l.radius / dlen * 1.001f, 1.0f);
+  if (!(sb < 0.5f)) return rec;
+  const v3 nd = normalized(dtl);
+  const float cb = sqrtf(fmaxf(1.0f - sb * sb, 0.0f));
+  const float dev = fmaxf(1.0f - cb, 0.0f);
+  rec.dlen = dlen;
+  rec.ndx = nd.x; rec.ndy = nd.y; rec.ndz = nd.z;
+  rec.spec_add = 1.0f - sqrt_rn(ang);
+  rec.near = near;
+  rec.cone_cos = 1.0f - dev - 4e-6f;
+  rec.cone_sin = sqrtf(fmaxf(1.0f - rec.cone_cos * rec.cone_cos, 0.0f) + 1e-7f) * 1.001f;
+  return rec;
+}
+
+static bool far_light_scene(const rfx_scene &s, const LightRec &rec)
+{
+  if (s.far_lights == 0 || s.lights.size() != 1 || !(rec.near > 0.0f)) return false;
+  if (s.far_lights == 2) return true;
+  const auto inside = [&](float v) { return fabsf(v) < rec.near; };
+  for (const HostSphere &h : s.spheres)
+    for (float v : {h.center.x - h.radius, h.center.x + h.radius, h.center.y - h.radius, h.center.y + h.radius,
+                    h.center.z - h.radius, h.center.z + h.radius})
+      if (!inside(v)) return false;
+  for (const HostTri &t : s.tris)
+    for (const v3 *v : {&t.v0, &t.v1, &t.v2})
+      if (!inside(v->x) || !inside(v->y) || !inside(v->z)) return false;
+  return true;
+}
+
+extern "C" int rfx_scene_set_far_lights(rfx_scene *s, int mode)
+{
+  if (!s || mode < 0 || mode > 2) return fail(RFX_ERR_ARG, "scene_set_far_lights: 0 (off), 1 (auto) or 2 (any extent)");
+  s->far_lights = mode;
+  return RFX_OK;
+}
+
+extern "C" int rfx_scene_far_light(const rfx_scene *s, int light, float terms[8])
+{
+  if (!s || light < 0 || light >= (int)s->lights.size()) return fail(RFX_ERR_ARG, "scene_far_light: no light %d", light);
+  const LightRec rec = far_light_terms(s->lights[light]);
+  if (terms)
+    for (float f : {rec.dlen, rec.ndx, rec.ndy, rec.ndz, rec.spec_add, rec.near, rec.cone_cos, rec.cone_sin}) *terms++ = f;
+  return far_light_scene(*s, rec) ? 1 : 0;
 }
 
 static OrderBox order_box_of(const rfx_scene &s)
@@ -917,7 +981,8 @@
       loc[o] = kind << 28 | (kind == 0 ? sph_dev[idx] : idx);
     }
   }
-  for (const HostLight &l : s->lights) lr.push_back({l.origin.x, l.origin.y, l.origin.z, l.radius, l.r, l.g, l.b, l.power});
+  for (const HostLight &l : s->lights) lr.push_back(far_light_terms(l));
+  d.far_light = !lr.empty() && far_light_scene(*s, lr[0]);
   for (const HostTexture &t : s->textures)
   {
     const bool empty = t.texels.empty();
diff --git a/reflaxman_amd/csrc/rfx_trace.h b/reflaxman_amd/csrc/rfx_trace.h
--- a/reflaxman_amd/csrc/rfx_trace.h
+++ b/reflaxman_amd/csrc/rfx_trace.h
@@ -143,6 +143,8 @@
   constexpr bool PLANES = (CFG & kCfgPlanes) != 0, PARK = MODE == kModePlain && !STATS && (CFG & kCfgPark) != 0;
   constexpr bool ONEL = (CFG & kCfgOneLight) != 0;
   constexpr bool TBVH = (CFG & kCfgTriBvh) != 0;
+  constexpr bool FARL = (CFG & kCfgFarLight) != 0;
+  static_assert(!FARL || (MODE == kModePlain || MODE == kModeSsaaLanes || MODE == kModeSsaaChunks), "far-light modes");
   RFX_WAVE_T0();
   __shared__ float lut[256];
   for (uint32_t i = threadIdx.x; i < 256; i += kWgThreads) lut[i] = (float)i / 255.0f;
@@ -207,8 +209,8 @@
       if (valid) rd = load_rd(P, pr * (uint64_t)ss2 + kk);
       const uint64_t *pm = RFX_PRIM_LANES && SMALL && CULL && !STATS && P.prim_mask
                                ? P.prim_mask + (size_t)kPrimStride * t8 : nullptr;
-      const col c = trace<STATS, CULL, MANYL, SMALL, PLANES, ONEL, TBVH>(S, eye, ray, P.depth, rd, lut, cnt, valid, pm,
-                                                                  P.prim_shadow != 0);
+      const col c = trace<STATS, CULL, MANYL, SMALL, PLANES, ONEL, TBVH, FARL>(S, eye, ray, P.depth, rd, lut, cnt, valid, pm,
+                                                                        P.prim_shadow != 0);
       {
 #ifdef RFX_LAUNDER_PARAMS
         const FrameParams &P = kernarg_params();
@@ -332,9 +334,8 @@
       if (valid) rd = load_rd(P, pr);
       const ParkTile park{P.park_after, P.queue, P.queue_count, P, wv, w8};
       const uint64_t *pm_tile = SMALL && CULL && !STATS && P.prim_mask ? P.prim_mask + (size_t)kPrimStride * t8 : nullptr;
-      const col c = trace_from<STATS, CULL, MANYL, SMALL, PLANES, PARK, ParkTile, ONEL, TBVH>(S, eye, ray, mkc(1.0f, 1.0f, 1.0f),
-                                                                  mkc(0.0f, 0.0f, 0.0f), 0, P.depth, rd, lut, cnt,
-                                                                  valid, park, parked, pm_tile);
+      const col c = trace_from<STATS, CULL, MANYL, SMALL, PLANES, PARK, ParkTile, ONEL, TBVH, FARL>(
+          S, eye, ray, mkc(1.0f, 1.0f, 1.0f), mkc(0.0f, 0.0f, 0.0f), 0, P.depth, rd, lut, cnt, valid, park, parked, pm_tile);
       out = cadd(mkc(0.0f, 0.0f, 0.0f), c);
     }
     else
@@ -429,6 +430,16 @@
     cfg &= ~kCfgTriBvh;
   }
 #endif
+  if (cfg & kCfgFarLight)
+  {
+    if constexpr (!STATS && RFX_FAR_LIGHT && (MODE == kModePlain || MODE == kModeSsaaLanes || MODE == kModeSsaaChunks))
+      switch (cfg & ~kCfgFarLight)
+      {
+        case 5 | kCfgOneLight: launch_one<STATS, MODE, 5 | kCfgOneLight | kCfgFarLight>(grid, S, P, st); return;
+        case 13 | kCfgOneLight: launch_one<STATS, MODE, 13 | kCfgOneLight | kCfgFarLight>(grid, S, P, st); return;
+      }
+    cfg &= ~kCfgFarLight;
+  }
   if (cfg & kCfgOneLight)
   {
     switch (cfg & ~kCfgOneLight)
diff --git a/reflaxman_amd/csrc/rfx_trace_plain_park.hip b/reflaxman_amd/csrc/rfx_trace_plain_park.hip
--- a/reflaxman_amd/csrc/rfx_trace_plain_park.hip
+++ b/reflaxman_amd/csrc/rfx_trace_plain_park.hip
@@ -15,7 +15,11 @@
 
 void launch_trace_plain_park(int cfg, dim3 grid, const DevScene &S, const FrameParams &P, hipStream_t st)
 {
-  switch (cfg & ~kCfgPark)
+#if RFX_FAR_LIGHT
+  if ((cfg & ~kCfgPark) == (5 | kCfgOneLight | kCfgFarLight))
+    return launch_park_one<5 | kCfgOneLight | kCfgFarLight>(grid, S, P, st);
+#endif
+  switch (cfg & ~(kCfgPark | kCfgFarLight))
   {
 #if RFX_TRI_BVH
     case 1 | kCfgTriBvh: launch_park_one<1 | kCfgTriBvh>(grid, S, P, st); break;
@@ -36,7 +40,7 @@
     case 13: launch_park_one<13>(grid, S, P, st); break;
     case 15: launch_park_one<15>(grid, S, P, st); break;
     default:
-      if (cfg & kCfgOneLight) launch_trace_plain_park(cfg & ~kCfgOneLight, grid, S, P, st);
+      if (cfg & kCfgOneLight) launch_trace_plain_park(cfg & ~(kCfgOneLight | kCfgFarLight), grid, S, P, st);
       break;
   }
 }
diff --git a/reflaxman_amd/csrc/rfx_types.h b/reflaxman_amd/csrc/rfx_types.h
--- a/reflaxman_amd/csrc/rfx_types.h
+++ b/reflaxman_amd/csrc/rfx_types.h
@@ -39,7 +39,10 @@
 constexpr int kBvhStack = 16;
 struct alignas(16) BvhNode { float lx[2], ly[2], lz[2], hx[2], hy[2], hz[2]; int32_t child[2]; float mt[2]; };
 struct alignas(16) PlaneGeo { float px, py, pz, nx, ny, nz; int32_t obj, dielectric; };
-struct alignas(16) LightRec { float ox, oy, oz, radius, r, g, b, power; };
+struct alignas(16) LightRec {
+  float ox, oy, oz, radius, r, g, b, power;
+  float dlen, ndx, ndy, ndz, spec_add, near, cone_cos, cone_sin;
+};
 struct alignas(16) TexRec { uint32_t offset, w, h, pad; };
 
 struct DevScene {
@@ -82,6 +85,7 @@
   int32_t n_tri_bvh;
   int32_t tri_bvh_depth;
   int32_t tri_bvh_narrow;
+  int32_t far_light;
 };
 
 constexpr int kLdsBvhWaves = 16, kLdsBvhStackSlots = 16;
@@ -142,5 +146,6 @@
 constexpr int kPrimLights = 4, kPrimStride = 1 + kPrimLights;
 constexpr int kCfgCull = 1, kCfgManyLights = 2, kCfgSmall = 4, kCfgPlanes = 8, kCfgPark = 16, kCfgOneLight = 32;
 constexpr int kCfgTriBvh = 64;
+constexpr int kCfgFarLight = 128;
 
 }
diff --git a/reflaxman_amd/render.py b/reflaxman_amd/render.py
--- a/reflaxman_amd/render.py
+++ b/reflaxman_amd/render.py
@@ -166,6 +166,15 @@
         leader, rows = np.zeros(n, np.int32), np.zeros((n, 6), np.float32)
         check(L.rfx_scene_tri_mates(self._h, leader.ctypes.data_as(_lib._i32p), _lib.fptr(rows)), "Scene.tri_mates")
         return (leader, rows) if plane else leader
+
+    def set_far_lights(self, mode: int):
+        check(_lib.load().rfx_scene_set_far_lights(self._h, int(mode)), "Scene.set_far_lights")
+        self._version += 1
+
+    def far_light(self, light: int = 0):
+        terms = np.zeros(8, np.float32)
+        chosen = check(_lib.load().rfx_scene_far_light(self._h, int(light), _lib.fptr(terms)), "Scene.far_light")
+        return bool(chosen), terms
 
     def addPlane(self, pos: Vector3, norm: Vector3, material: Material) -> Plane:
         obj = check(_lib.load().rfx_scene_add_plane(self._h, farr(Vector3(*pos)), farr(Vector3(*norm)), material.type,
@@ -726,6 +735,12 @@
         check(_lib.load().rfx_kat_powf(self._h, _lib.fptr(xy), xy.shape[0], _lib.fptr(out)), "rfx_kat_powf")
         return out
 
+    def kat_far_light(self, points: np.ndarray) -> np.ndarray:
+        pts = np.ascontiguousarray(points, np.float32).reshape(-1, 3)
+        out = np.zeros((pts.shape[0], 8), np.float32)
+        check(_lib.load().rfx_kat_far_light(self._h, _lib.fptr(pts), pts.shape[0], _lib.fptr(out)), "rfx_kat_far_light")
+        return out
+
     def kat_powf_cube(self):
         counts = (C.c_uint64 * 2)()
         check(_lib.load().rfx_kat_powf_cube(self._h, counts), "rfx_kat_powf_cube")
```

Result: faster. 14370 Mrays/s (median of 6 runs) (+5.0%).
